# a16z/jolt

Hardware: AMD Instinct MI355X
Metric: prover trace cycles/sec (sha3-shaped synthetic trace, sumcheck + HyperKZG hot path) (higher is better)
Workload: dtype u256 (BN254 Fr / Fq, 8x u32 Montgomery limbs; integer, bit-exact)

## Files before the change

### jolt_amd/csrc/rw_matrix.hip

```cpp
#include <algorithm>
#include <vector>

#include "ctx.hpp"
#include "ints.hpp"
#include "onehot.hpp"
#include "poly_kernels.hip.h"

using namespace jolt;

int32_t jolt_internal_table_new(jolt_ctx* ctx, size_t len, jolt_table** out);
int32_t jolt_internal_bind(jolt_ctx* ctx, jolt_table* const* tables, size_t k, const Fr& r, int32_t order);
int32_t jolt_internal_eq_levels(jolt_ctx* ctx, const Fr* r, size_t n, const Fr& scale, std::vector<jolt_table*>* levels);
int32_t jolt_internal_ensure_scratch(jolt_ctx* ctx, size_t partials, size_t results);

namespace {

constexpr uint64_t kNoAccess = 0xFFFFFFFFFFFFFFFFull;

struct RwArrays {
    uint64_t* key;
    uint64_t *prev_u, *next_u;
    Fr *prev_f, *next_f;
    Fr *val, *ra;
    Fr* wa;
};

__device__ __forceinline__ uint32_t lower_bound_near(const uint64_t* __restrict__ a, uint32_t n, uint64_t x, uint32_t hint) {
    uint32_t lo, hi;
    if (a[hint] < x) {
        uint32_t prev = hint, step = 1;
        hi = n;
        for (;;) {
            const uint32_t probe = prev + step;
            if (probe >= n || probe < prev) break;
            if (a[probe] < x) { prev = probe; step <<= 1; }
            else { hi = probe; break; }
        }
        lo = prev + 1;
    } else {
        uint32_t next = hint, step = 1;
        lo = 0;
        for (;;) {
            if (next < step) break;
            const uint32_t probe = next - step;
            if (a[probe] >= x) { next = probe; step <<= 1; }
            else { lo = probe + 1; break; }
        }
        hi = next;
    }
    while (lo < hi) {
        const uint32_t mid = (lo + hi) >> 1;
        if (a[mid] < x) lo = mid + 1;
        else hi = mid;
    }
    return lo;
}

__device__ __forceinline__ Fr bind_pair(const Fr& lo, const Fr& hi, const Fr& r, int shifted) {
    return shifted ? jolt::bind_pair<true>(lo, hi, r) : jolt::bind_pair<false>(lo, hi, r);
}
__device__ __forceinline__ Fr slope_term(const Fr& val, const Fr& inc, const Fr& gamma) { return add(val, mul(gamma, add(inc, val))); }

__global__ __launch_bounds__(kBlock) void k_rw_access_flags(const uint64_t* __restrict__ addresses, uint32_t cycles, uint64_t* __restrict__ flags) {
    uint32_t j = blockIdx.x * kBlock + threadIdx.x;
    if (j < cycles) flags[j] = addresses[j] != kNoAccess ? 1ull : 0ull;
}
__global__ __launch_bounds__(kBlock) void k_rw_build(const uint64_t* __restrict__ addresses, const uint64_t* __restrict__ pre, const uint64_t* __restrict__ post,
                                                     uint32_t cycles, const uint64_t* __restrict__ pos, RwArrays o) {
    uint32_t j = blockIdx.x * kBlock + threadIdx.x;
    if (j >= cycles || addresses[j] == kNoAccess) return;
    const uint32_t p = (uint32_t)pos[j];
    o.key[p] = ((uint64_t)j << 32) | (uint32_t)addresses[j];
    o.prev_u[p] = pre[j];
    o.next_u[p] = post[j];
    st_fr(o.val + p, fr_from_u64(pre[j]));
    st_fr(o.ra + p, Fr::one());
}

struct RegCells {
    uint32_t col[3];
    uint64_t prev[3], next[3], val[3];
    uint32_t ra_kind[3];
    uint32_t wa[3];
    uint32_t len;
};
__device__ __forceinline__ RegCells reg_cells(uint32_t rs1, uint64_t rs1_val, uint32_t rs2, uint64_t rs2_val, uint32_t rd, uint64_t rd_pre, uint64_t rd_post) {
    RegCells c;
    c.len = 0;
    if (rs1 != kColdIdx) { c.col[0] = rs1; c.prev[0] = rs1_val; c.next[0] = rs1_val; c.val[0] = rs1_val; c.ra_kind[0] = 1; c.wa[0] = 0; c.len = 1; }
    if (rs2 != kColdIdx) {
        if (c.len && c.col[0] == rs2) c.ra_kind[0] = 3;
        else { const uint32_t k = c.len++; c.col[k] = rs2; c.prev[k] = rs2_val; c.next[k] = rs2_val; c.val[k] = rs2_val; c.ra_kind[k] = 2; c.wa[k] = 0; }
    }
    if (rd != kColdIdx) {
        uint32_t f = 0;
        while (f < c.len && c.col[f] != rd) ++f;
        if (f < c.len) { c.wa[f] = 1; c.next[f] = rd_post; }
        else { const uint32_t k = c.len++; c.col[k] = rd; c.prev[k] = rd_pre; c.next[k] = rd_post; c.val[k] = rd_pre; c.ra_kind[k] = 0; c.wa[k] = 1; }
    }
    return c;
}
__global__ __launch_bounds__(kBlock) void k_reg_count(const uint8_t* __restrict__ idx, uint32_t wide, uint32_t cycles, uint64_t* __restrict__ flags) {
    const uint32_t j = blockIdx.x * kBlock + threadIdx.x;
    if (j >= cycles) return;
    const uint32_t rs1 = hot_load(hot_col(idx, 0, wide), j, wide), rs2 = hot_load(hot_col(idx, cycles, wide), j, wide), rd = hot_load(hot_col(idx, 2 * (size_t)cycles, wide), j, wide);
    uint32_t count = rs1 != kColdIdx ? 1u : 0u;
    if (rs2 != kColdIdx && rs2 != rs1) count += 1;
    if (rd != kColdIdx && rd != rs1 && rd != rs2) count += 1;
    flags[j] = count;
}
__global__ __launch_bounds__(kBlock) void k_reg_build(const uint8_t* __restrict__ idx, uint32_t wide, const uint64_t* __restrict__ rs1_val, const uint64_t* __restrict__ rs2_val,
                                                      const uint64_t* __restrict__ rd_pre, const uint64_t* __restrict__ rd_post, uint32_t cycles, const uint64_t* __restrict__ pos,
                                                      Fr gamma, Fr gamma2, RwArrays o) {
    const uint32_t j = blockIdx.x * kBlock + threadIdx.x;
    if (j >= cycles) return;
    const uint32_t rs1 = hot_load(hot_col(idx, 0, wide), j, wide), rs2 = hot_load(hot_col(idx, cycles, wide), j, wide), rd = hot_load(hot_col(idx, 2 * (size_t)cycles, wide), j, wide);
    RegCells c = reg_cells(rs1, rs1_val[j], rs2, rs2_val[j], rd, rd_pre[j], rd_post[j]);
    uint32_t ord[3] = {0, 1, 2};
    for (uint32_t a = 0; a < c.len; ++a)
        for (uint32_t b = a + 1; b < c.len; ++b)
            if (c.col[ord[b]] < c.col[ord[a]]) { const uint32_t t = ord[a]; ord[a] = ord[b]; ord[b] = t; }
    const uint32_t p0 = (uint32_t)pos[j];
    for (uint32_t a = 0; a < c.len; ++a) {
        const uint32_t k = ord[a], p = p0 + a;
        o.key[p] = ((uint64_t)j << 32) | c.col[k];
        o.prev_u[p] = c.prev[k];
        o.next_u[p] = c.next[k];
        st_fr(o.val + p, fr_from_u64(c.val[k]));
        const Fr ra = c.ra_kind[k] == 0 ? Fr::zero() : (c.ra_kind[k] == 1 ? gamma : (c.ra_kind[k] == 2 ? gamma2 : add(gamma, gamma2)));
        st_fr(o.ra + p, ra);
        st_fr(o.wa + p, c.wa[k] ? Fr::one() : Fr::zero());
    }
}

constexpr int kScanItems = 4;
__global__ __launch_bounds__(kBlock) void k_scan_blocks(const uint64_t* __restrict__ in, uint32_t n, uint64_t* __restrict__ out, uint64_t* __restrict__ block_sums) {
    __shared__ uint64_t sm[kBlock];
    const uint32_t base = (blockIdx.x * kBlock + threadIdx.x) * kScanItems;
    uint64_t v[kScanItems], local = 0;
#pragma unroll
    for (int k = 0; k < kScanItems; ++k) {
        v[k] = base + k < n ? in[base + k] : 0ull;
        local += v[k];
    }
    sm[threadIdx.x] = local;
    __syncthreads();
    for (int off = 1; off < kBlock; off <<= 1) {
        uint64_t t = (int)threadIdx.x >= off ? sm[threadIdx.x - off] : 0ull;
        __syncthreads();
        sm[threadIdx.x] += t;
        __syncthreads();
    }
    uint64_t run = sm[threadIdx.x] - local;
#pragma unroll
    for (int k = 0; k < kScanItems; ++k) {
        if (base + k < n) out[base + k] = run;
        run += v[k];
    }
    if (threadIdx.x == kBlock - 1) block_sums[blockIdx.x] = sm[threadIdx.x];
}
__global__ __launch_bounds__(kBlock) void k_scan_sums(uint64_t* __restrict__ sums, uint32_t nblocks, uint64_t* __restrict__ total) {
    __shared__ uint64_t sm[kBlock];
    __shared__ uint64_t carry;
    if (threadIdx.x == 0) carry = 0;
    __syncthreads();
    for (uint32_t base = 0; base < nblocks; base += kBlock) {
        const uint32_t i = base + threadIdx.x;
        const uint64_t v = i < nblocks ? sums[i] : 0ull;
        sm[threadIdx.x] = v;
        __syncthreads();
        for (int off = 1; off < kBlock; off <<= 1) {
            uint64_t t = (int)threadIdx.x >= off ? sm[threadIdx.x - off] : 0ull;
            __syncthreads();
            sm[threadIdx.x] += t;
            __syncthreads();
        }
        if (i < nblocks) sums[i] = carry + sm[threadIdx.x] - v;
        __syncthreads();
        if (threadIdx.x == kBlock - 1) carry += sm[threadIdx.x];
        __syncthreads();
    }
    if (threadIdx.x == 0) total[0] = carry;
}
__global__ __launch_bounds__(kBlock) void k_scan_add(uint64_t* __restrict__ out, uint32_t n, const uint64_t* __restrict__ block_sums) {
    const uint32_t base = (blockIdx.x * kBlock + threadIdx.x) * kScanItems;
    const uint64_t add_ = block_sums[blockIdx.x];
#pragma unroll
    for (int k = 0; k < kScanItems; ++k)
        if (base + k < n) out[base + k] += add_;
}

__global__ __launch_bounds__(kBlock) void k_rw_cycle_match(const uint64_t* __restrict__ key, uint32_t n, uint32_t* __restrict__ sib_lb, uint32_t* __restrict__ matched,
                                                           uint64_t* __restrict__ flags) {
    uint32_t i = blockIdx.x * kBlock + threadIdx.x;
    if (i >= n) return;
    const uint64_t k = key[i], want = k ^ (1ull << 32);
    const uint32_t lb = lower_bound_near(key, n, want, i);
    const bool m = lb < n && key[lb] == want;
    const bool even = ((k >> 32) & 1) == 0;
    sib_lb[i] = lb;
    matched[i] = m ? 1u : 0u;
    flags[i] = ((even || !m) ? 1ull : 0ull) | ((even && m) ? (1ull << 32) : 0ull);
}

template <bool REG>
__global__ __launch_bounds__(kBlock) void k_rw_cycle_round(RwArrays a, uint32_t n, const uint32_t* __restrict__ sib_lb, const uint32_t* __restrict__ matched,
                                                           const Fr* __restrict__ inc, const Fr* __restrict__ e_out, const Fr* __restrict__ e_in, int in_bits, Fr gamma,
                                                           Fr* __restrict__ partials) {
    Fr acc[2] = {Fr::zero(), Fr::zero()};
    const uint32_t stride = gridDim.x * kBlock;
    for (uint32_t i = blockIdx.x * kBlock + threadIdx.x; i < n; i += stride) {
        const uint64_t k = a.key[i];
        const uint32_t row = (uint32_t)(k >> 32);
        const bool even = (row & 1) == 0, m = matched[i] != 0;
        if (!even && m) continue;
        const uint32_t pair = row >> 1;
        const Fr inc0 = ld_fr(inc + 2 * (size_t)pair), inc1 = sub(ld_fr(inc + 2 * (size_t)pair + 1), inc0);
        const Fr ra = ld_fr(a.ra + i), val = ld_fr(a.val + i);
        Fr q0, q1;
        if constexpr (REG) {
            const Fr wa = ld_fr(a.wa + i);
            if (even) {
                Fr ra_slope, wa_slope, val_slope;
                if (m) {
                    const uint32_t o = sib_lb[i];
                    ra_slope = sub(ld_fr(a.ra + o), ra);
                    wa_slope = sub(ld_fr(a.wa + o), wa);
                    val_slope = sub(ld_fr(a.val + o), val);
                } else {
                    ra_slope = neg(ra);
                    wa_slope = neg(wa);
                    val_slope = sub(fr_from_u64(a.next_u[i]), val);
                }
                q0 = add(mul(ra, val), mul(wa, add(val, inc0)));
                q1 = add(mul(ra_slope, val_slope), mul(wa_slope, add(val_slope, inc1)));
            } else {
                const Fr val_slope = sub(val, fr_from_u64(a.prev_u[i]));
                q0 = Fr::zero();
                q1 = add(mul(ra, val_slope), mul(wa, add(val_slope, inc1)));
            }
        } else if (even) {
            Fr ra_slope, val_slope;
            if (m) {
                const uint32_t o = sib_lb[i];
                ra_slope = sub(ld_fr(a.ra + o), ra);
                val_slope = sub(ld_fr(a.val + o), val);
            } else {
                ra_slope = neg(ra);
                val_slope = sub(fr_from_u64(a.next_u[i]), val);
            }
            q0 = mul(ra, slope_term(val, inc0, gamma));
            q1 = mul(ra_slope, slope_term(val_slope, inc1, gamma));
        } else {
            q0 = Fr::zero();
            q1 = mul(ra, slope_term(sub(val, fr_from_u64(a.prev_u[i])), inc1, gamma));
        }
        const Fr head = mul(ld_fr(e_out + (pair >> in_bits)), ld_fr(e_in + (pair & ((1u << in_bits) - 1))));
        acc[0] = add(acc[0], mul(head, q0));
        acc[1] = add(acc[1], mul(head, q1));
    }
    block_reduce_store<2>(acc, partials);
}

template <bool REG>
__global__ __launch_bounds__(kBlock) void k_rw_cycle_bind(RwArrays a, uint32_t n, const uint32_t* __restrict__ sib_lb, const uint32_t* __restrict__ matched,
                                                          const uint64_t* __restrict__ scan, Fr r, int shifted, RwArrays o) {
    uint32_t i = blockIdx.x * kBlock + threadIdx.x;
    if (i >= n) return;
    const uint64_t k = a.key[i];
    const uint32_t row = (uint32_t)(k >> 32), col = (uint32_t)k;
    const bool even = (row & 1) == 0, m = matched[i] != 0;
    if (!even && m) return;
    const uint64_t gkey = (uint64_t)(row & ~1u) << 32;
    const uint32_t gs = lower_bound_near(a.key, n, gkey, i), os = lower_bound_near(a.key, n, gkey | (1ull << 32), i);
    const uint64_t s_gs = gs < n ? scan[gs] : 0;
    const uint32_t out_base = (uint32_t)s_gs, m_gs = (uint32_t)(s_gs >> 32);
    const uint32_t lb = sib_lb[i];
    uint32_t pos;
    if (even) pos = out_base + (i - gs) + (lb - os) - ((uint32_t)(scan[i] >> 32) - m_gs);
    else pos = out_base + (i - os) + (lb - gs) - ((lb < n ? (uint32_t)(scan[lb] >> 32) : 0u) - m_gs);
    const Fr ra = ld_fr(a.ra + i), val = ld_fr(a.val + i);
    Fr nra, nval;
    uint64_t np, nn;
    auto lerp = [&](const Fr& lo, const Fr& hi) { return bind_pair(lo, hi, r, shifted); };
    if (even && m) {
        nra = lerp(ra, ld_fr(a.ra + lb));
        nval = lerp(val, ld_fr(a.val + lb));
        np = a.prev_u[i];
        nn = a.next_u[lb];
    } else if (even) {
        nra = lerp(ra, Fr::zero());
        nval = lerp(val, fr_from_u64(a.next_u[i]));
        np = a.prev_u[i];
        nn = a.next_u[i];
    } else {
        nra = lerp(Fr::zero(), ra);
        nval = lerp(fr_from_u64(a.prev_u[i]), val);
        np = a.prev_u[i];
        nn = a.next_u[i];
    }
    o.key[pos] = ((uint64_t)(row >> 1) << 32) | col;
    o.prev_u[pos] = np;
    o.next_u[pos] = nn;
    st_fr(o.ra + pos, nra);
    st_fr(o.val + pos, nval);
    if constexpr (REG) {
        const Fr wa = ld_fr(a.wa + i);
        st_fr(o.wa + pos, (even && m) ? lerp(wa, ld_fr(a.wa + lb)) : (even ? lerp(wa, Fr::zero()) : lerp(Fr::zero(), wa)));
    }
}

__global__ __launch_bounds__(kBlock) void k_rw_to_address_major(RwArrays a, uint32_t n) {
    uint32_t i = blockIdx.x * kBlock + threadIdx.x;
    if (i >= n) return;
    a.key[i] = (uint32_t)a.key[i];
    st_fr(a.prev_f + i, fr_from_u64(a.prev_u[i]));
    st_fr(a.next_f + i, fr_from_u64(a.next_u[i]));
}

__device__ __forceinline__ bool adr_partner(const uint64_t* __restrict__ key, uint32_t n, uint32_t i, uint32_t& other) {
    const uint64_t c = key[i];
    if ((c & 1) == 0) { other = i + 1; return i + 1 < n && key[i + 1] == c + 1; }
    other = i - 1;
    return i > 0 && key[i - 1] == c - 1;
}
__global__ __launch_bounds__(kBlock) void k_rw_address_flags(const uint64_t* __restrict__ key, uint32_t n, uint64_t* __restrict__ flags) {
    uint32_t i = blockIdx.x * kBlock + threadIdx.x;
    if (i >= n) return;
    uint32_t o;
    const bool m = adr_partner(key, n, i, o);
    flags[i] = ((key[i] & 1) == 0 || !m) ? 1ull : 0ull;
}
__global__ __launch_bounds__(kBlock) void k_rw_address_round(RwArrays a, uint32_t n, const Fr* __restrict__ val_init, const Fr* __restrict__ inc_scalar, Fr eq_eval,
                                                             Fr gamma, Fr* __restrict__ partials) {
    Fr acc[2] = {Fr::zero(), Fr::zero()};
    const Fr inc = ld_fr(inc_scalar);
    const uint32_t stride = gridDim.x * kBlock;
    for (uint32_t i = blockIdx.x * kBlock + threadIdx.x; i < n; i += stride) {
        uint32_t o;
        const bool m = adr_partner(a.key, n, i, o);
        const uint64_t c = a.key[i];
        const bool even = (c & 1) == 0;
        if (!even && m) continue;
        const Fr ra = ld_fr(a.ra + i), val = ld_fr(a.val + i);
        Fr s0, s2;
        if (even) {
            Fr ra2, val2;
            if (m) {
                const Fr ora = ld_fr(a.ra + o), oval = ld_fr(a.val + o);
                ra2 = sub(add(ora, ora), ra);
                val2 = sub(add(oval, oval), val);
            } else {
                const Fr cp = ld_fr(val_init + (c | 1));
                ra2 = neg(ra);
                val2 = sub(add(cp, cp), val);
            }
            s0 = mul(mul(eq_eval, ra), slope_term(val, inc, gamma));
            s2 = mul(mul(eq_eval, ra2), slope_term(val2, inc, gamma));
        } else {
            const Fr cp = ld_fr(val_init + (c & ~1ull));
            s0 = Fr::zero();
            s2 = mul(mul(eq_eval, add(ra, ra)), slope_term(sub(add(val, val), cp), inc, gamma));
        }
        acc[0] = add(acc[0], s0);
        acc[1] = add(acc[1], s2);
    }
    block_reduce_store<2>(acc, partials);
}
__global__ __launch_bounds__(kBlock) void k_rw_address_bind(RwArrays a, uint32_t n, const Fr* __restrict__ val_init, const uint64_t* __restrict__ scan, Fr r, int shifted,
                                                            RwArrays o) {
    uint32_t i = blockIdx.x * kBlock + threadIdx.x;
    if (i >= n) return;
    uint32_t p;
    const bool m = adr_partner(a.key, n, i, p);
    const uint64_t c = a.key[i];
    const bool even = (c & 1) == 0;
    if (!even && m) return;
    const uint32_t pos = (uint32_t)scan[i];
    auto lerp = [&](const Fr& lo, const Fr& hi) { return bind_pair(lo, hi, r, shifted); };
    const Fr ra = ld_fr(a.ra + i), val = ld_fr(a.val + i), pv = ld_fr(a.prev_f + i), nx = ld_fr(a.next_f + i);
    Fr nra, nval, npv, nnx;
    if (even && m) {
        nra = lerp(ra, ld_fr(a.ra + p));
        nval = lerp(val, ld_fr(a.val + p));
        npv = lerp(pv, ld_fr(a.prev_f + p));
        nnx = lerp(nx, ld_fr(a.next_f + p));
    } else if (even) {
        const Fr cp = ld_fr(val_init + (c | 1));
        nra = lerp(ra, Fr::zero());
        nval = lerp(val, cp);
        npv = lerp(pv, cp);
        nnx = lerp(nx, cp);
    } else {
        const Fr cp = ld_fr(val_init + (c & ~1ull));
        nra = lerp(Fr::zero(), ra);
        nval = lerp(cp, val);
        npv = lerp(cp, pv);
        nnx = lerp(cp, nx);
    }
    o.key[pos] = c >> 1;
    st_fr(o.ra + pos, nra);
    st_fr(o.val + pos, nval);
    st_fr(o.prev_f + pos, npv);
    st_fr(o.next_f + pos, nnx);
}

}

struct jolt_rw_matrix {
    jolt_ctx* ctx = nullptr;
    size_t log_t = 0, log_k = 0, round = 0;
    uint32_t n = 0, cap = 0;
    void* block = nullptr;
    RwArrays st[2];
    int cur = 0;
    uint32_t *sib_lb = nullptr, *matched = nullptr;
    uint64_t *flags = nullptr, *scan = nullptr, *block_sums = nullptr, *total = nullptr;
    uint64_t* h_total = nullptr;
    bool match_valid = false;
    bool registers = false;
    bool hold_row = false;
    std::vector<Fr> reg_ra, reg_wa, reg_val;
    Fr inc_scalar;
    jolt_table *inc = nullptr, *val_init = nullptr;
    Fr gamma;
    std::vector<Fr> w;
    Fr current_scalar;
    size_t out_len = 0, in_len = 0, e_out_bits = 0, e_in_bits = 0;
    std::vector<jolt_table*> e_out_cache, e_in_cache;
};

static int32_t rw_scan(jolt_rw_matrix* m, uint32_t n) {
    jolt_ctx* ctx = m->ctx;
    const uint32_t per = kBlock * kScanItems, nblocks = std::max<uint32_t>(1, (n + per - 1) / per);
    hipLaunchKernelGGL(k_scan_blocks, dim3(nblocks), dim3(kBlock), 0, ctx->stream, (const uint64_t*)m->flags, n, m->scan, m->block_sums);
    hipLaunchKernelGGL(k_scan_sums, dim3(1), dim3(kBlock), 0, ctx->stream, m->block_sums, nblocks, m->total);
    hipLaunchKernelGGL(k_scan_add, dim3(nblocks), dim3(kBlock), 0, ctx->stream, m->scan, n, (const uint64_t*)m->block_sums);
    JOLT_HIP_TRY(ctx, hipGetLastError());
    return JOLT_OK;
}
static int32_t rw_read_total(jolt_rw_matrix* m, uint32_t* out) {
    jolt_ctx* ctx = m->ctx;
    JOLT_HIP_TRY(ctx, hipMemcpyAsync(m->h_total, m->total, 8, hipMemcpyDeviceToHost, ctx->stream));
    JOLT_HIP_TRY(ctx, hipStreamSynchronize(ctx->stream));
    *out = (uint32_t)*m->h_total;
    return JOLT_OK;
}
static unsigned rw_grid(uint32_t n) { return std::max<unsigned>(1, (n + kBlock - 1) / kBlock); }
constexpr uint32_t kRwRoundMult = 4;

extern "C" int32_t jolt_rw_matrix_destroy(jolt_rw_matrix* m) {
    if (!m) return JOLT_OK;
    jolt_ctx* ctx = m->ctx;
    if (m->block) jolt_internal_dev_free(ctx, m->block);
    if (m->h_total) (void)hipHostFree(m->h_total);
    if (m->inc) jolt_table_free(ctx, m->inc);
    if (m->val_init) jolt_table_free(ctx, m->val_init);
    for (jolt_table* t : m->e_out_cache) jolt_table_free(ctx, t);
    for (jolt_table* t : m->e_in_cache) jolt_table_free(ctx, t);
    delete m;
    return JOLT_OK;
}

static int32_t rw_create_impl(jolt_ctx* ctx, const uint64_t* addresses, const uint64_t* pre_values, const uint64_t* post_values, bool resident, uint32_t resident_cap,
                              size_t cycles, const jolt_table* inc, const jolt_table* val_init, const jolt_fr_t* tau_low, const jolt_fr_t* gamma, jolt_rw_matrix** out) {
    if (!ctx || !addresses || !pre_values || !post_values || !inc || !val_init || !tau_low || !gamma || !out) return JOLT_ERR_INVALID_ARG;
    if (cycles < 2 || (cycles & (cycles - 1)) || cycles > ((size_t)1 << 31) || inc->len != cycles) return JOLT_ERR_SIZE_MISMATCH;
    const size_t K = val_init->len;
    if (K == 0 || (K & (K - 1)) || K > ((size_t)1 << 32)) return JOLT_ERR_SIZE_MISMATCH;
    for (size_t j = 0; j < cycles && !resident; ++j)
        if (addresses[j] != kNoAccess && addresses[j] >= K) { ctx->last_error = "RAM address outside the address space"; return JOLT_ERR_INVALID_ARG; }
    jolt_rw_matrix* m = new (std::nothrow) jolt_rw_matrix();
    if (!m) return JOLT_ERR_OOM;
    m->ctx = ctx;
    while (((size_t)1 << m->log_t) < cycles) m->log_t++;
    while (((size_t)1 << m->log_k) < K) m->log_k++;
    m->gamma = fr_from_abi(gamma);
    m->w.resize(m->log_t);
    for (size_t i = 0; i < m->log_t; ++i) m->w[i] = fr_from_abi(&tau_low[i]);
    m->current_scalar = Fr::one();
    int32_t s = fr_is_canonical(m->gamma) ? JOLT_OK : JOLT_ERR_INVALID_ARG;
    for (size_t i = 0; i < m->log_t && s == JOLT_OK; ++i) if (!fr_is_canonical(m->w[i])) s = JOLT_ERR_INVALID_ARG;
    const size_t split = m->log_t / 2, head_len = m->log_t - 1;
    m->out_len = std::min(split, head_len);
    m->in_len = head_len - m->out_len;
    m->e_out_bits = m->out_len;
    m->e_in_bits = m->in_len;
    if (s == JOLT_OK) s = jolt_internal_eq_levels(ctx, m->w.data(), m->out_len, Fr::one(), &m->e_out_cache);
    if (s == JOLT_OK) s = jolt_internal_eq_levels(ctx, m->w.data() + m->out_len, m->in_len, Fr::one(), &m->e_in_cache);
    if (s == JOLT_OK) s = jolt_table_clone(ctx, inc, &m->inc);
    if (s == JOLT_OK) s = jolt_table_clone(ctx, val_init, &m->val_init);
    const uint32_t T = (uint32_t)cycles;
    uint32_t cap = resident_cap;
    for (size_t j = 0; j < cycles && !resident; ++j) cap += addresses[j] != kNoAccess;
    m->cap = std::max<uint32_t>(cap, 1);
    const size_t scan_len = std::max<size_t>(T, m->cap);
    size_t off = 0;
    auto take = [&](size_t bytes) { size_t o = off; off += (bytes + 255) & ~(size_t)255; return o; };
    size_t o_up = take(resident ? 256 : 3 * cycles * 8);
    size_t o_st[2][8];
    for (int b = 0; b < 2; ++b) {
        o_st[b][0] = take((size_t)m->cap * 8); o_st[b][1] = take((size_t)m->cap * 8); o_st[b][2] = take((size_t)m->cap * 8);
        o_st[b][3] = take((size_t)m->cap * 32); o_st[b][4] = take((size_t)m->cap * 32); o_st[b][5] = take((size_t)m->cap * 32); o_st[b][6] = take((size_t)m->cap * 32);
        o_st[b][7] = take(256);
    }
    const size_t o_sib = take((size_t)m->cap * 4), o_match = take((size_t)m->cap * 4), o_flags = take(scan_len * 8), o_scan = take(scan_len * 8),
                 o_bs = take(((scan_len + kBlock * kScanItems - 1) / (kBlock * kScanItems) + 1) * 8), o_total = take(256);
    if (s == JOLT_OK) s = jolt_internal_dev_alloc(ctx, off, &m->block);
    if (s == JOLT_OK && hipHostMalloc((void**)&m->h_total, 64, hipHostMallocDefault) != hipSuccess) s = JOLT_ERR_HIP;
    if (s != JOLT_OK) { jolt_rw_matrix_destroy(m); return s; }
    char* base = (char*)m->block;
    for (int b = 0; b < 2; ++b) {
        m->st[b].key = (uint64_t*)(base + o_st[b][0]); m->st[b].prev_u = (uint64_t*)(base + o_st[b][1]); m->st[b].next_u = (uint64_t*)(base + o_st[b][2]);
        m->st[b].prev_f = (Fr*)(base + o_st[b][3]); m->st[b].next_f = (Fr*)(base + o_st[b][4]); m->st[b].val = (Fr*)(base + o_st[b][5]); m->st[b].ra = (Fr*)(base + o_st[b][6]);
        m->st[b].wa = (Fr*)(base + o_st[b][7]);
    }
    m->sib_lb = (uint32_t*)(base + o_sib); m->matched = (uint32_t*)(base + o_match); m->flags = (uint64_t*)(base + o_flags); m->scan = (uint64_t*)(base + o_scan);
    m->block_sums = (uint64_t*)(base + o_bs); m->total = (uint64_t*)(base + o_total);
    const uint64_t *d_addr = addresses, *d_pre = pre_values, *d_post = post_values;
    hipError_t e = hipSuccess;
    if (!resident) {
        uint64_t* up = (uint64_t*)(base + o_up);
        d_addr = up; d_pre = up + cycles; d_post = up + 2 * cycles;
        e = hipMemcpyAsync(up, addresses, cycles * 8, hipMemcpyHostToDevice, ctx->stream);
        if (e == hipSuccess) e = hipMemcpyAsync(up + cycles, pre_values, cycles * 8, hipMemcpyHostToDevice, ctx->stream);
        if (e == hipSuccess) e = hipMemcpyAsync(up + 2 * cycles, post_values, cycles * 8, hipMemcpyHostToDevice, ctx->stream);
    }
    if (e == hipSuccess) {
        hipLaunchKernelGGL(k_rw_access_flags, dim3(rw_grid(T)), dim3(kBlock), 0, ctx->stream, (const uint64_t*)d_addr, T, m->flags);
        e = hipGetLastError();
    }
    if (e == hipSuccess) s = rw_scan(m, T);
    if (e == hipSuccess && s == JOLT_OK) {
        hipLaunchKernelGGL(k_rw_build, dim3(rw_grid(T)), dim3(kBlock), 0, ctx->stream, (const uint64_t*)d_addr, (const uint64_t*)d_pre, (const uint64_t*)d_post, T,
                           (const uint64_t*)m->scan, m->st[0]);
        e = hipGetLastError();
    }
    if (e == hipSuccess && !resident) e = hipStreamSynchronize(ctx->stream);
    if (e != hipSuccess || s != JOLT_OK) {
        if (e != hipSuccess) { ctx->last_error = std::string("rw matrix: ") + hipGetErrorString(e); s = JOLT_ERR_HIP; }
        jolt_rw_matrix_destroy(m);
        return s;
    }
    m->n = cap;
    *out = m;
    return JOLT_OK;
}
extern "C" int32_t jolt_rw_matrix_create(jolt_ctx* ctx, const uint64_t* addresses, const uint64_t* pre_values, const uint64_t* post_values, size_t cycles,
                                         const jolt_table* inc, const jolt_table* val_init, const jolt_fr_t* tau_low, const jolt_fr_t* gamma, jolt_rw_matrix** out) {
    return rw_create_impl(ctx, addresses, pre_values, post_values, false, 0, cycles, inc, val_init, tau_low, gamma, out);
}
__global__ __launch_bounds__(kBlock) void k_rw_count_accesses(const uint64_t* __restrict__ addresses, uint32_t cycles, uint64_t K, uint32_t* __restrict__ counters) {
    __shared__ uint32_t s_hit[kBlock / 64], s_bad[kBlock / 64];
    uint32_t hit = 0, bad = 0;
    for (uint32_t j = blockIdx.x * kBlock + threadIdx.x; j < cycles; j += gridDim.x * kBlock) {
        const uint64_t a = addresses[j];
        hit += a != kNoAccess ? 1u : 0u;
        bad += (a != kNoAccess && a >= K) ? 1u : 0u;
    }
    for (int off = 32; off >= 1; off >>= 1) {
        hit += __shfl_xor(hit, off, 64);
        bad += __shfl_xor(bad, off, 64);
    }
    if ((threadIdx.x & 63) == 0) { s_hit[threadIdx.x >> 6] = hit; s_bad[threadIdx.x >> 6] = bad; }
    __syncthreads();
    if (threadIdx.x == 0) {
        uint32_t h = 0, b = 0;
        for (int w = 0; w < kBlock / 64; ++w) { h += s_hit[w]; b += s_bad[w]; }
        if (h) atomicAdd(&counters[0], h);
        if (b) atomicAdd(&counters[1], b);
    }
}
extern "C" int32_t jolt_rw_matrix_create_resident(jolt_ctx* ctx, const jolt_ints* addresses, const jolt_ints* pre_values, const jolt_ints* post_values,
                                                  const jolt_table* inc, const jolt_table* val_init, const jolt_fr_t* tau_low, const jolt_fr_t* gamma, jolt_rw_matrix** out) {
    if (!ctx || !addresses || !pre_values || !post_values || !val_init || !out) return JOLT_ERR_INVALID_ARG;
    if (addresses->kind != JOLT_INT_U64 || pre_values->kind != JOLT_INT_U64 || post_values->kind != JOLT_INT_U64) return JOLT_ERR_INVALID_ARG;
    const size_t cycles = addresses->count;
    if (pre_values->count != cycles || post_values->count != cycles) return JOLT_ERR_SIZE_MISMATCH;
    if (cycles < 2 || cycles > ((size_t)1 << 31)) return JOLT_ERR_SIZE_MISMATCH;
    uint32_t* d_counters = nullptr;
    JOLT_TRY(jolt_internal_dev_alloc(ctx, 256, (void**)&d_counters));
    uint32_t h_counters[2] = {0, 0};
    hipError_t e = hipMemsetAsync(d_counters, 0, 8, ctx->stream);
    if (e == hipSuccess) {
        hipLaunchKernelGGL(k_rw_count_accesses, dim3(std::min<uint32_t>(rw_grid((uint32_t)cycles), (uint32_t)ctx->num_cus * 8)), dim3(kBlock), 0, ctx->stream, (const uint64_t*)addresses->data, (uint32_t)cycles,
                           (uint64_t)val_init->len, d_counters);
        e = hipGetLastError();
    }
    if (e == hipSuccess) e = hipMemcpyAsync(h_counters, d_counters, 8, hipMemcpyDeviceToHost, ctx->stream);
    if (e == hipSuccess) e = hipStreamSynchronize(ctx->stream);
    jolt_internal_dev_free(ctx, d_counters);
    if (e != hipSuccess) { ctx->last_error = std::string("rw matrix: ") + hipGetErrorString(e); return JOLT_ERR_HIP; }
    if (h_counters[1]) { ctx->last_error = "RAM address outside the address space"; return JOLT_ERR_INVALID_ARG; }
    return rw_create_impl(ctx, (const uint64_t*)addresses->data, (const uint64_t*)pre_values->data, (const uint64_t*)post_values->data, true, h_counters[0], cycles, inc,
                          val_init, tau_low, gamma, out);
}

static int32_t rw_ingest(jolt_rw_matrix* m, const Fr& r) {
    jolt_ctx* ctx = m->ctx;
    const int shifted = fr_low_limbs_zero(r) ? 1 : 0;
    RwArrays &a = m->st[m->cur], &o = m->st[1 - m->cur];
    if (m->round < m->log_t) {
        if (m->n) {
            if (!m->match_valid) {
                hipLaunchKernelGGL(k_rw_cycle_match, dim3(rw_grid(m->n)), dim3(kBlock), 0, ctx->stream, (const uint64_t*)a.key, m->n, m->sib_lb, m->matched, m->flags);
                JOLT_HIP_TRY(ctx, hipGetLastError());
            }
            JOLT_TRY(rw_scan(m, m->n));
            if (m->registers)
                hipLaunchKernelGGL(k_rw_cycle_bind<true>, dim3(rw_grid(m->n)), dim3(kBlock), 0, ctx->stream, a, m->n, (const uint32_t*)m->sib_lb, (const uint32_t*)m->matched,
                                   (const uint64_t*)m->scan, r, shifted, o);
            else
                hipLaunchKernelGGL(k_rw_cycle_bind<false>, dim3(rw_grid(m->n)), dim3(kBlock), 0, ctx->stream, a, m->n, (const uint32_t*)m->sib_lb, (const uint32_t*)m->matched,
                                   (const uint64_t*)m->scan, r, shifted, o);
            JOLT_HIP_TRY(ctx, hipGetLastError());
            JOLT_TRY(rw_read_total(m, &m->n));
            m->cur = 1 - m->cur;
        }
        m->match_valid = false;
        JOLT_TRY(jolt_internal_bind(ctx, &m->inc, 1, r, JOLT_ORDER_LOW_TO_HIGH));
        {
            const size_t nvar = m->log_t;
            size_t current_index = nvar - m->round;
            const Fr p = m->w[current_index - 1], prod = mul(p, r);
            m->current_scalar = mul(m->current_scalar, add(add(sub(sub(Fr::one(), p), r), prod), prod));
            current_index -= 1;
            if (nvar / 2 < current_index && m->e_in_bits > 0) m->e_in_bits -= 1;
            else if (0 < current_index && m->e_out_bits > 0) m->e_out_bits -= 1;
        }
        if (m->round == m->log_t - 1 && m->hold_row) {
        } else if (m->round == m->log_t - 1 && m->registers) {
            const size_t K = (size_t)1 << m->log_k;
            m->reg_ra.assign(K, Fr::zero());
            m->reg_wa.assign(K, Fr::zero());
            m->reg_val.assign(K, Fr::zero());
            const uint32_t n = m->n;
            if (n > K) { ctx->last_error = "registers matrix: more cells than registers after the cycle rounds"; return JOLT_ERR_INVALID_ARG; }
            std::vector<uint64_t> key(n);
            std::vector<Fr> ra(n), wa(n), val(n);
            const RwArrays& c = m->st[m->cur];
            hipError_t first = hipSuccess;
            auto copy = [&](void* dst, const void* src, size_t bytes) {
                const hipError_t e = hipMemcpyAsync(dst, src, bytes, hipMemcpyDeviceToHost, ctx->stream);
                if (first == hipSuccess) first = e;
            };
            if (n) {
                copy(key.data(), c.key, (size_t)n * 8);
                copy(ra.data(), c.ra, (size_t)n * sizeof(Fr));
                copy(wa.data(), c.wa, (size_t)n * sizeof(Fr));
                copy(val.data(), c.val, (size_t)n * sizeof(Fr));
            }
            copy(&m->inc_scalar, m->inc->data(), sizeof(Fr));
            const hipError_t sync = hipStreamSynchronize(ctx->stream);
            JOLT_HIP_TRY(ctx, first);
            JOLT_HIP_TRY(ctx, sync);
            for (uint32_t i = 0; i < n; ++i) {
                const uint32_t col = (uint32_t)key[i];
                if ((key[i] >> 32) != 0 || col >= K) { ctx->last_error = "registers matrix: a cell outside the single bound row"; return JOLT_ERR_INVALID_ARG; }
                m->reg_ra[col] = ra[i]; m->reg_wa[col] = wa[i]; m->reg_val[col] = val[i];
            }
        } else if (m->round == m->log_t - 1 && m->n) {
            hipLaunchKernelGGL(k_rw_to_address_major, dim3(rw_grid(m->n)), dim3(kBlock), 0, ctx->stream, m->st[m->cur], m->n);
            JOLT_HIP_TRY(ctx, hipGetLastError());
        }
    } else if (m->registers) {
        for (std::vector<Fr>* t : {&m->reg_ra, &m->reg_wa, &m->reg_val}) {
            const size_t half = t->size() / 2;
            for (size_t y = 0; y < half; ++y) (*t)[y] = add((*t)[2 * y], mul(r, sub((*t)[2 * y + 1], (*t)[2 * y])));
            t->resize(half);
        }
    } else {
        if (m->n) {
            hipLaunchKernelGGL(k_rw_address_flags, dim3(rw_grid(m->n)), dim3(kBlock), 0, ctx->stream, (const uint64_t*)a.key, m->n, m->flags);
            JOLT_HIP_TRY(ctx, hipGetLastError());
            JOLT_TRY(rw_scan(m, m->n));
            hipLaunchKernelGGL(k_rw_address_bind, dim3(rw_grid(m->n)), dim3(kBlock), 0, ctx->stream, a, m->n, (const Fr*)m->val_init->data(), (const uint64_t*)m->scan, r,
                               shifted, o);
            JOLT_HIP_TRY(ctx, hipGetLastError());
            JOLT_TRY(rw_read_total(m, &m->n));
            m->cur = 1 - m->cur;
        }
        JOLT_TRY(jolt_internal_bind(ctx, &m->val_init, 1, r, JOLT_ORDER_LOW_TO_HIGH));
    }
    m->round += 1;
    return JOLT_OK;
}

extern "C" int32_t jolt_rw_matrix_prove_round(jolt_rw_matrix* m, const jolt_fr_t* bind, jolt_fr_t* evals_out, jolt_fr_t* aux_out) {
    if (!m || !evals_out) return JOLT_ERR_INVALID_ARG;
    jolt_ctx* ctx = m->ctx;
    if (m->registers) { ctx->last_error = "a registers handle: use jolt_registers_rw_prove_round (this entry point ignores the wa column)"; return JOLT_ERR_INVALID_ARG; }
    if (bind) {
        Fr r = fr_from_abi(bind);
        JOLT_REQUIRE(ctx, fr_is_canonical(r), "bind challenge is not a canonical Fr");
        if (m->round >= m->log_t + m->log_k) { ctx->last_error = "rw matrix already fully bound"; return JOLT_ERR_INVALID_ARG; }
        JOLT_TRY(rw_ingest(m, r));
    }
    if (m->round >= m->log_t + m->log_k) { ctx->last_error = "prove_round on a fully bound rw matrix"; return JOLT_ERR_INVALID_ARG; }
    const int grid = (int)std::max<uint32_t>(1, std::min<uint32_t>((m->n + kBlock - 1) / kBlock, (uint32_t)ctx->num_cus * kRwRoundMult));
    JOLT_TRY(jolt_internal_ensure_scratch(ctx, (size_t)grid * 2 + 8, 8));
    RwArrays& a = m->st[m->cur];
    Fr zero = Fr::zero();
    if (m->round < m->log_t) {
        if (m->n && !m->match_valid) {
            hipLaunchKernelGGL(k_rw_cycle_match, dim3(rw_grid(m->n)), dim3(kBlock), 0, ctx->stream, (const uint64_t*)a.key, m->n, m->sib_lb, m->matched, m->flags);
            JOLT_HIP_TRY(ctx, hipGetLastError());
            m->match_valid = true;
        }
        hipLaunchKernelGGL(k_rw_cycle_round<false>, dim3(grid), dim3(kBlock), 0, ctx->stream, a, m->n, (const uint32_t*)m->sib_lb, (const uint32_t*)m->matched,
                           (const Fr*)m->inc->data(), (const Fr*)m->e_out_cache[m->e_out_bits]->data(), (const Fr*)m->e_in_cache[m->e_in_bits]->data(), (int)m->e_in_bits,
                           m->gamma, ctx->d_partials);
        if (aux_out) {
            fr_to_abi(&aux_out[0], m->current_scalar);
            fr_to_abi(&aux_out[1], m->w[m->log_t - m->round - 1]);
            fr_to_abi(&aux_out[2], zero);
        }
    } else {
        hipLaunchKernelGGL(k_rw_address_round, dim3(grid), dim3(kBlock), 0, ctx->stream, a, m->n, (const Fr*)m->val_init->data(), (const Fr*)m->inc->data(),
                           m->current_scalar, m->gamma, ctx->d_partials);
        if (aux_out) for (int k = 0; k < 3; ++k) fr_to_abi(&aux_out[k], zero);
    }
    JOLT_HIP_TRY(ctx, hipGetLastError());
    hipLaunchKernelGGL(k_reduce_partials, dim3(1), dim3(kBlock), 0, ctx->stream, (const Fr*)ctx->d_partials, grid, 2, ctx->d_results);
    JOLT_HIP_TRY(ctx, hipGetLastError());
    JOLT_HIP_TRY(ctx, hipMemcpyAsync(ctx->h_results, ctx->d_results, 2 * sizeof(Fr), hipMemcpyDeviceToHost, ctx->stream));
    JOLT_HIP_TRY(ctx, hipStreamSynchronize(ctx->stream));
    std::memcpy(evals_out, ctx->h_results, 2 * sizeof(Fr));
    return JOLT_OK;
}

extern "C" int32_t jolt_rw_matrix_finish(jolt_rw_matrix* m, const jolt_fr_t* bind) {
    if (!m || !bind) return JOLT_ERR_INVALID_ARG;
    Fr r = fr_from_abi(bind);
    JOLT_REQUIRE(m->ctx, fr_is_canonical(r), "bind challenge is not a canonical Fr");
    if (m->round + 1 != m->log_t + m->log_k) { m->ctx->last_error = "finish_rounds before the last round"; return JOLT_ERR_INVALID_ARG; }
    return rw_ingest(m, r);
}

extern "C" int32_t jolt_rw_matrix_final_values(jolt_rw_matrix* m, jolt_fr_t* out) {
    if (!m || !out) return JOLT_ERR_INVALID_ARG;
    jolt_ctx* ctx = m->ctx;
    if (m->registers) { ctx->last_error = "a registers handle: use jolt_registers_rw_final_values (no val_init column here)"; return JOLT_ERR_INVALID_ARG; }
    if (m->round != m->log_t + m->log_k) return JOLT_ERR_NOT_FULLY_BOUND;
    Fr vals[3];
    if (m->n) {
        JOLT_HIP_TRY(ctx, hipMemcpyAsync(&vals[0], m->st[m->cur].ra, sizeof(Fr), hipMemcpyDeviceToHost, ctx->stream));
        JOLT_HIP_TRY(ctx, hipMemcpyAsync(&vals[1], m->st[m->cur].val, sizeof(Fr), hipMemcpyDeviceToHost, ctx->stream));
    } else {
        vals[0] = Fr::zero();
        JOLT_HIP_TRY(ctx, hipMemcpyAsync(&vals[1], m->val_init->data(), sizeof(Fr), hipMemcpyDeviceToHost, ctx->stream));
    }
    JOLT_HIP_TRY(ctx, hipMemcpyAsync(&vals[2], m->inc->data(), sizeof(Fr), hipMemcpyDeviceToHost, ctx->stream));
    JOLT_HIP_TRY(ctx, hipStreamSynchronize(ctx->stream));
    for (int k = 0; k < 3; ++k) fr_to_abi(&out[k], vals[k]);
    fr_to_abi(&out[3], m->current_scalar);
    return JOLT_OK;
}

extern "C" int32_t jolt_rw_matrix_len(const jolt_rw_matrix* m, size_t* entries) {
    if (!m || !entries) return JOLT_ERR_INVALID_ARG;
    *entries = m->n;
    return JOLT_OK;
}

extern "C" int32_t jolt_rw_matrix_hold_row(jolt_rw_matrix* m) {
    if (!m || m->round != 0) return JOLT_ERR_INVALID_ARG;
    m->hold_row = true;
    return JOLT_OK;
}
extern "C" int32_t jolt_rw_matrix_bind(jolt_rw_matrix* m, const jolt_fr_t* bind) {
    if (!m || !bind) return JOLT_ERR_INVALID_ARG;
    const Fr r = fr_from_abi(bind);
    JOLT_REQUIRE(m->ctx, fr_is_canonical(r), "bind challenge is not a canonical Fr");
    if (m->round >= m->log_t + m->log_k || (m->hold_row && m->round >= m->log_t)) { m->ctx->last_error = "rw matrix already bound"; return JOLT_ERR_INVALID_ARG; }
    return rw_ingest(m, r);
}
extern "C" int32_t jolt_rw_matrix_export_row(jolt_rw_matrix* m, size_t cap, uint64_t* cols, uint64_t* prev, uint64_t* next, jolt_fr_t* val, jolt_fr_t* ra, jolt_fr_t* wa,
                                             jolt_fr_t* inc_out, jolt_fr_t* scalar_out, size_t* n_out) {
    if (!m || !cols || !prev || !next || !val || !ra || !inc_out || !scalar_out || !n_out || (m->registers && !wa)) return JOLT_ERR_INVALID_ARG;
    jolt_ctx* ctx = m->ctx;
    if (!m->hold_row || m->round != m->log_t) { ctx->last_error = "export_row: a held matrix after its last cycle round"; return JOLT_ERR_INVALID_ARG; }
    const uint32_t n = m->n;
    *n_out = n;
    if (n > cap) return JOLT_ERR_SIZE_MISMATCH;
    const RwArrays& a = m->st[m->cur];
    std::vector<uint64_t> key(n);
    hipError_t first = hipSuccess;
    auto copy = [&](void* dst, const void* src, size_t bytes) {
        const hipError_t e = bytes ? hipMemcpyAsync(dst, src, bytes, hipMemcpyDeviceToHost, ctx->stream) : hipSuccess;
        if (first == hipSuccess) first = e;
    };
    copy(key.data(), a.key, (size_t)n * 8);
    copy(prev, a.prev_u, (size_t)n * 8);
    copy(next, a.next_u, (size_t)n * 8);
    copy(val, a.val, (size_t)n * sizeof(Fr));
    copy(ra, a.ra, (size_t)n * sizeof(Fr));
    if (m->registers) copy(wa, a.wa, (size_t)n * sizeof(Fr));
    Fr inc;
    copy(&inc, m->inc->data(), sizeof(Fr));
    const hipError_t sync = hipStreamSynchronize(ctx->stream);
    JOLT_HIP_TRY(ctx, first);
    JOLT_HIP_TRY(ctx, sync);
    for (uint32_t i = 0; i < n; ++i) {
        if (key[i] >> 32) { ctx->last_error = "export_row: a cell outside the single bound row"; return JOLT_ERR_INVALID_ARG; }
        cols[i] = (uint32_t)key[i];
    }
    fr_to_abi(inc_out, inc);
    fr_to_abi(scalar_out, m->current_scalar);
    return JOLT_OK;
}

extern "C" int32_t jolt_rw_matrix_create_merged(jolt_ctx* ctx, int32_t registers, size_t log_rows, size_t log_k, size_t n, const uint64_t* rows, const uint64_t* cols,
                                                const uint64_t* prev, const uint64_t* next, const jolt_fr_t* val, const jolt_fr_t* ra, const jolt_fr_t* wa, const jolt_fr_t* inc,
                                                const jolt_table* val_init, const jolt_fr_t* w, const jolt_fr_t* scalar, const jolt_fr_t* gamma, jolt_rw_matrix** out) {
    if (!ctx || !inc || !w || !scalar || !gamma || !out || (n && (!rows || !cols || !prev || !next || !val || !ra))) return JOLT_ERR_INVALID_ARG;
    if ((registers && n && !wa) || (!registers && !val_init)) return JOLT_ERR_INVALID_ARG;
    if (log_rows < 1 || log_rows > 16 || log_k > 32 || n >= ((size_t)1 << 31)) return JOLT_ERR_UNSUPPORTED;
    if (registers && log_k > 8) return JOLT_ERR_SIZE_MISMATCH;
    if (!registers && val_init->len != ((size_t)1 << log_k)) return JOLT_ERR_SIZE_MISMATCH;
    std::vector<uint64_t> key(n);
    for (size_t i = 0; i < n; ++i) {
        if (rows[i] >> log_rows || cols[i] >> log_k) { ctx->last_error = "merged rw matrix: a cell outside the matrix"; return JOLT_ERR_INVALID_ARG; }
        key[i] = (rows[i] << 32) | cols[i];
        if (i && key[i] <= key[i - 1]) { ctx->last_error = "merged rw matrix: cells must come in (row, column) order"; return JOLT_ERR_INVALID_ARG; }
    }
    jolt_rw_matrix* m = new (std::nothrow) jolt_rw_matrix();
    if (!m) return JOLT_ERR_OOM;
    m->ctx = ctx;
    m->registers = registers != 0;
    m->log_t = log_rows;
    m->log_k = log_k;
    m->gamma = fr_from_abi(gamma);
    m->current_scalar = fr_from_abi(scalar);
    m->w.resize(log_rows);
    for (size_t i = 0; i < log_rows; ++i) m->w[i] = fr_from_abi(&w[i]);
    int32_t s = fr_is_canonical(m->gamma) && fr_is_canonical(m->current_scalar) ? JOLT_OK : JOLT_ERR_INVALID_ARG;
    for (size_t i = 0; i < log_rows && s == JOLT_OK; ++i) if (!fr_is_canonical(m->w[i])) s = JOLT_ERR_INVALID_ARG;
    const size_t split = m->log_t / 2, head_len = m->log_t - 1;
    m->out_len = std::min(split, head_len);
    m->in_len = head_len - m->out_len;
    m->e_out_bits = m->out_len;
    m->e_in_bits = m->in_len;
    if (s == JOLT_OK) s = jolt_internal_eq_levels(ctx, m->w.data(), m->out_len, Fr::one(), &m->e_out_cache);
    if (s == JOLT_OK) s = jolt_internal_eq_levels(ctx, m->w.data() + m->out_len, m->in_len, Fr::one(), &m->e_in_cache);
    if (s == JOLT_OK) s = jolt_table_upload(ctx, inc, (size_t)1 << log_rows, &m->inc);
    if (s == JOLT_OK && !registers) s = jolt_table_clone(ctx, val_init, &m->val_init);
    m->cap = (uint32_t)std::max<size_t>(n, 1);
    const size_t scan_len = std::max<size_t>((size_t)1 << log_rows, m->cap);
    size_t off = 0;
    auto take = [&](size_t bytes) { size_t o = off; off += (bytes + 255) & ~(size_t)255; return o; };
    size_t o_st[2][8];
    for (int b = 0; b < 2; ++b) {
        o_st[b][0] = take((size_t)m->cap * 8); o_st[b][1] = take((size_t)m->cap * 8); o_st[b][2] = take((size_t)m->cap * 8);
        o_st[b][3] = take(registers ? 256 : (size_t)m->cap * 32); o_st[b][4] = take(registers ? 256 : (size_t)m->cap * 32);
        o_st[b][5] = take((size_t)m->cap * 32); o_st[b][6] = take((size_t)m->cap * 32); o_st[b][7] = take(registers ? (size_t)m->cap * 32 : 256);
    }
    const size_t o_sib = take((size_t)m->cap * 4), o_match = take((size_t)m->cap * 4), o_flags = take(scan_len * 8), o_scan = take(scan_len * 8),
                 o_bs = take(((scan_len + kBlock * kScanItems - 1) / (kBlock * kScanItems) + 1) * 8), o_total = take(256);
    if (s == JOLT_OK) s = jolt_internal_dev_alloc(ctx, off, &m->block);
    if (s == JOLT_OK && hipHostMalloc((void**)&m->h_total, 64, hipHostMallocDefault) != hipSuccess) s = JOLT_ERR_HIP;
    if (s != JOLT_OK) { jolt_rw_matrix_destroy(m); return s; }
    char* base = (char*)m->block;
    for (int b = 0; b < 2; ++b) {
        m->st[b].key = (uint64_t*)(base + o_st[b][0]); m->st[b].prev_u = (uint64_t*)(base + o_st[b][1]); m->st[b].next_u = (uint64_t*)(base + o_st[b][2]);
        m->st[b].prev_f = registers ? nullptr : (Fr*)(base + o_st[b][3]); m->st[b].next_f = registers ? nullptr : (Fr*)(base + o_st[b][4]);
        m->st[b].val = (Fr*)(base + o_st[b][5]); m->st[b].ra = (Fr*)(base + o_st[b][6]); m->st[b].wa = (Fr*)(base + o_st[b][7]);
    }
    m->sib_lb = (uint32_t*)(base + o_sib); m->matched = (uint32_t*)(base + o_match); m->flags = (uint64_t*)(base + o_flags); m->scan = (uint64_t*)(base + o_scan);
    m->block_sums = (uint64_t*)(base + o_bs); m->total = (uint64_t*)(base + o_total);
    hipError_t first = hipSuccess;
    auto up = [&](void* dst, const void* src, size_t bytes) {
        const hipError_t e = bytes ? hipMemcpyAsync(dst, src, bytes, hipMemcpyHostToDevice, ctx->stream) : hipSuccess;
        if (first == hipSuccess) first = e;
    };
    up(m->st[0].key, key.data(), n * 8);
    up(m->st[0].prev_u, prev, n * 8);
    up(m->st[0].next_u, next, n * 8);
    up(m->st[0].val, val, n * sizeof(Fr));
    up(m->st[0].ra, ra, n * sizeof(Fr));
    if (registers) up(m->st[0].wa, wa, n * sizeof(Fr));
    const hipError_t sync = hipStreamSynchronize(ctx->stream);
    if (first != hipSuccess || sync != hipSuccess) {
        ctx->last_error = std::string("merged rw matrix: ") + hipGetErrorString(first != hipSuccess ? first : sync);
        jolt_rw_matrix_destroy(m);
        return JOLT_ERR_HIP;
    }
    m->n = (uint32_t)n;
    *out = m;
    return JOLT_OK;
}

extern "C" int32_t jolt_rw_matrix_download(jolt_rw_matrix* m, uint64_t* rows, uint64_t* cols, jolt_fr_t* val, jolt_fr_t* ra, jolt_fr_t* prev, jolt_fr_t* next) {
    if (!m || !rows || !cols || !val || !ra || !prev || !next) return JOLT_ERR_INVALID_ARG;
    jolt_ctx* ctx = m->ctx;
    if (m->registers) { ctx->last_error = "a registers handle: use jolt_registers_rw_download (no prev / next field columns here)"; return JOLT_ERR_INVALID_ARG; }
    const uint32_t n = m->n;
    if (!n) return JOLT_OK;
    const RwArrays& a = m->st[m->cur];
    const bool address_major = m->round >= m->log_t;
    std::vector<uint64_t> key(n), pu(n), nu(n);
    JOLT_HIP_TRY(ctx, hipMemcpyAsync(key.data(), a.key, (size_t)n * 8, hipMemcpyDeviceToHost, ctx->stream));
    JOLT_HIP_TRY(ctx, hipMemcpyAsync(val, a.val, (size_t)n * 32, hipMemcpyDeviceToHost, ctx->stream));
    JOLT_HIP_TRY(ctx, hipMemcpyAsync(ra, a.ra, (size_t)n * 32, hipMemcpyDeviceToHost, ctx->stream));
    if (address_major) {
        JOLT_HIP_TRY(ctx, hipMemcpyAsync(prev, a.prev_f, (size_t)n * 32, hipMemcpyDeviceToHost, ctx->stream));
        JOLT_HIP_TRY(ctx, hipMemcpyAsync(next, a.next_f, (size_t)n * 32, hipMemcpyDeviceToHost, ctx->stream));
    } else {
        JOLT_HIP_TRY(ctx, hipMemcpyAsync(pu.data(), a.prev_u, (size_t)n * 8, hipMemcpyDeviceToHost, ctx->stream));
        JOLT_HIP_TRY(ctx, hipMemcpyAsync(nu.data(), a.next_u, (size_t)n * 8, hipMemcpyDeviceToHost, ctx->stream));
    }
    JOLT_HIP_TRY(ctx, hipStreamSynchronize(ctx->stream));
    for (uint32_t i = 0; i < n; ++i) {
        rows[i] = address_major ? 0 : key[i] >> 32;
        cols[i] = address_major ? key[i] : (uint32_t)key[i];
        if (!address_major) {
            Fr p = fr_from_u64(pu[i]), q = fr_from_u64(nu[i]);
            fr_to_abi(&prev[i], p);
            fr_to_abi(&next[i], q);
        }
    }
    return JOLT_OK;
}

extern "C" int32_t jolt_registers_rw_create(jolt_ctx* ctx, const jolt_onehot* regs, const jolt_ints* rs1_val, const jolt_ints* rs2_val, const jolt_ints* rd_pre,
                                            const jolt_ints* rd_post, const jolt_table* inc, const jolt_fr_t* r_cycle, const jolt_fr_t* gamma, jolt_rw_matrix** out) {
    if (!ctx || !regs || !rs1_val || !rs2_val || !rd_pre || !rd_post || !inc || !r_cycle || !gamma || !out) return JOLT_ERR_INVALID_ARG;
    if (regs->n_polys != 3) { ctx->last_error = "registers columns: a hot-index source with the three columns rs1, rs2, rd"; return JOLT_ERR_INVALID_ARG; }
    const size_t cycles = regs->cycles, K = regs->k;
    for (const jolt_ints* c : {rs1_val, rs2_val, rd_pre, rd_post}) {
        if (c->kind != JOLT_INT_U64) return JOLT_ERR_INVALID_ARG;
        if (c->count != cycles) return JOLT_ERR_SIZE_MISMATCH;
    }
    if (cycles < 2 || (cycles & (cycles - 1)) || cycles > ((size_t)1 << 30) || inc->len != cycles) return JOLT_ERR_SIZE_MISMATCH;
    if (K == 0 || (K & (K - 1)) || K > 256) return JOLT_ERR_SIZE_MISMATCH;
    jolt_rw_matrix* m = new (std::nothrow) jolt_rw_matrix();
    if (!m) return JOLT_ERR_OOM;
    m->ctx = ctx;
    m->registers = true;
    while (((size_t)1 << m->log_t) < cycles) m->log_t++;
    while (((size_t)1 << m->log_k) < K) m->log_k++;
    m->gamma = fr_from_abi(gamma);
    m->w.resize(m->log_t);
    for (size_t i = 0; i < m->log_t; ++i) m->w[i] = fr_from_abi(&r_cycle[i]);
    m->current_scalar = Fr::one();
    int32_t s = fr_is_canonical(m->gamma) ? JOLT_OK : JOLT_ERR_INVALID_ARG;
    for (size_t i = 0; i < m->log_t && s == JOLT_OK; ++i) if (!fr_is_canonical(m->w[i])) s = JOLT_ERR_INVALID_ARG;
    const size_t split = m->log_t / 2, head_len = m->log_t - 1;
    m->out_len = std::min(split, head_len);
    m->in_len = head_len - m->out_len;
    m->e_out_bits = m->out_len;
    m->e_in_bits = m->in_len;
    if (s == JOLT_OK) s = jolt_internal_eq_levels(ctx, m->w.data(), m->out_len, Fr::one(), &m->e_out_cache);
    if (s == JOLT_OK) s = jolt_internal_eq_levels(ctx, m->w.data() + m->out_len, m->in_len, Fr::one(), &m->e_in_cache);
    if (s == JOLT_OK) s = jolt_table_clone(ctx, inc, &m->inc);
    const uint32_t T = (uint32_t)cycles;
    const size_t scan_len0 = T;
    uint64_t *d_flags0 = nullptr;
    if (s == JOLT_OK) s = jolt_internal_dev_alloc(ctx, (2 * scan_len0 + ((scan_len0 + kBlock * kScanItems - 1) / (kBlock * kScanItems) + 1) + 32) * 8, (void**)&d_flags0);
    if (s == JOLT_OK && hipHostMalloc((void**)&m->h_total, 64, hipHostMallocDefault) != hipSuccess) s = JOLT_ERR_HIP;
    if (s != JOLT_OK) { if (d_flags0) jolt_internal_dev_free(ctx, d_flags0); jolt_rw_matrix_destroy(m); return s; }
    m->flags = d_flags0; m->scan = d_flags0 + scan_len0; m->block_sums = m->scan + scan_len0; m->total = m->block_sums + ((scan_len0 + kBlock * kScanItems - 1) / (kBlock * kScanItems) + 1);
    hipLaunchKernelGGL(k_reg_count, dim3(rw_grid(T)), dim3(kBlock), 0, ctx->stream, (const uint8_t*)regs->idx, regs->wide, T, m->flags);
    s = hipGetLastError() == hipSuccess ? rw_scan(m, T) : JOLT_ERR_HIP;
    uint32_t cap = 0;
    if (s == JOLT_OK) s = rw_read_total(m, &cap);
    if (s != JOLT_OK) { jolt_internal_dev_free(ctx, d_flags0); m->flags = m->scan = m->block_sums = m->total = nullptr; jolt_rw_matrix_destroy(m); return s; }
    m->cap = std::max<uint32_t>(cap, 1);
    const size_t scan_len = std::max<size_t>(T, m->cap);
    size_t off = 0;
    auto take = [&](size_t bytes) { size_t o = off; off += (bytes + 255) & ~(size_t)255; return o; };
    size_t o_st[2][6];
    for (int b = 0; b < 2; ++b) {
        o_st[b][0] = take((size_t)m->cap * 8); o_st[b][1] = take((size_t)m->cap * 8); o_st[b][2] = take((size_t)m->cap * 8);
        o_st[b][3] = take((size_t)m->cap * 32); o_st[b][4] = take((size_t)m->cap * 32); o_st[b][5] = take((size_t)m->cap * 32);
    }
    const size_t o_sib = take((size_t)m->cap * 4), o_match = take((size_t)m->cap * 4), o_flags = take(scan_len * 8), o_scan = take(scan_len * 8),
                 o_bs = take(((scan_len + kBlock * kScanItems - 1) / (kBlock * kScanItems) + 1) * 8), o_total = take(256);
    s = jolt_internal_dev_alloc(ctx, off, &m->block);
    if (s != JOLT_OK) { jolt_internal_dev_free(ctx, d_flags0); m->flags = m->scan = m->block_sums = m->total = nullptr; jolt_rw_matrix_destroy(m); return s; }
    char* base = (char*)m->block;
    for (int b = 0; b < 2; ++b) {
        m->st[b].key = (uint64_t*)(base + o_st[b][0]); m->st[b].prev_u = (uint64_t*)(base + o_st[b][1]); m->st[b].next_u = (uint64_t*)(base + o_st[b][2]);
        m->st[b].val = (Fr*)(base + o_st[b][3]); m->st[b].ra = (Fr*)(base + o_st[b][4]); m->st[b].wa = (Fr*)(base + o_st[b][5]);
        m->st[b].prev_f = nullptr; m->st[b].next_f = nullptr;
    }
    const uint64_t* pos = m->scan;
    hipLaunchKernelGGL(k_reg_build, dim3(rw_grid(T)), dim3(kBlock), 0, ctx->stream, (const uint8_t*)regs->idx, regs->wide, (const uint64_t*)rs1_val->data, (const uint64_t*)rs2_val->data,
                       (const uint64_t*)rd_pre->data, (const uint64_t*)rd_post->data, T, pos, m->gamma, mul(m->gamma, m->gamma), m->st[0]);
    hipError_t e = hipGetLastError();
    jolt_internal_dev_free(ctx, d_flags0);
    m->sib_lb = (uint32_t*)(base + o_sib); m->matched = (uint32_t*)(base + o_match); m->flags = (uint64_t*)(base + o_flags); m->scan = (uint64_t*)(base + o_scan);
    m->block_sums = (uint64_t*)(base + o_bs); m->total = (uint64_t*)(base + o_total);
    if (e != hipSuccess) { ctx->last_error = std::string("registers matrix: ") + hipGetErrorString(e); jolt_rw_matrix_destroy(m); return JOLT_ERR_HIP; }
    m->n = cap;
    *out = m;
    return JOLT_OK;
}

extern "C" int32_t jolt_registers_rw_prove_round(jolt_rw_matrix* m, const jolt_fr_t* bind, jolt_fr_t* evals_out, jolt_fr_t* aux_out) {
    if (!m || !evals_out || !m->registers) return JOLT_ERR_INVALID_ARG;
    jolt_ctx* ctx = m->ctx;
    if (bind) {
        Fr r = fr_from_abi(bind);
        JOLT_REQUIRE(ctx, fr_is_canonical(r), "bind challenge is not a canonical Fr");
        if (m->round >= m->log_t + m->log_k) { ctx->last_error = "registers matrix already fully bound"; return JOLT_ERR_INVALID_ARG; }
        JOLT_TRY(rw_ingest(m, r));
    }
    if (m->round >= m->log_t + m->log_k) { ctx->last_error = "prove_round on a fully bound registers matrix"; return JOLT_ERR_INVALID_ARG; }
    const Fr zero = Fr::zero();
    for (int k = 0; k < 4; ++k) fr_to_abi(&evals_out[k], zero);
    if (aux_out) for (int k = 0; k < 3; ++k) fr_to_abi(&aux_out[k], zero);
    if (m->round < m->log_t) {
        const int grid = (int)std::max<uint32_t>(1, std::min<uint32_t>((m->n + kBlock - 1) / kBlock, (uint32_t)ctx->num_cus * kRwRoundMult));
        JOLT_TRY(jolt_internal_ensure_scratch(ctx, (size_t)grid * 2 + 8, 8));
        RwArrays& a = m->st[m->cur];
        if (m->n && !m->match_valid) {
            hipLaunchKernelGGL(k_rw_cycle_match, dim3(rw_grid(m->n)), dim3(kBlock), 0, ctx->stream, (const uint64_t*)a.key, m->n, m->sib_lb, m->matched, m->flags);
            JOLT_HIP_TRY(ctx, hipGetLastError());
            m->match_valid = true;
        }
        hipLaunchKernelGGL(k_rw_cycle_round<true>, dim3(grid), dim3(kBlock), 0, ctx->stream, a, m->n, (const uint32_t*)m->sib_lb, (const uint32_t*)m->matched, (const Fr*)m->inc->data(),
                           (const Fr*)m->e_out_cache[m->e_out_bits]->data(), (const Fr*)m->e_in_cache[m->e_in_bits]->data(), (int)m->e_in_bits, m->gamma, ctx->d_partials);
        JOLT_HIP_TRY(ctx, hipGetLastError());
        hipLaunchKernelGGL(k_reduce_partials, dim3(1), dim3(kBlock), 0, ctx->stream, (const Fr*)ctx->d_partials, grid, 2, ctx->d_results);
        JOLT_HIP_TRY(ctx, hipGetLastError());
        JOLT_HIP_TRY(ctx, hipMemcpyAsync(ctx->h_results, ctx->d_results, 2 * sizeof(Fr), hipMemcpyDeviceToHost, ctx->stream));
        JOLT_HIP_TRY(ctx, hipStreamSynchronize(ctx->stream));
        std::memcpy(evals_out, ctx->h_results, 2 * sizeof(Fr));
        if (aux_out) {
            fr_to_abi(&aux_out[0], m->current_scalar);
            fr_to_abi(&aux_out[1], m->w[m->log_t - m->round - 1]);
        }
        return JOLT_OK;
    }
    Fr ev[4] = {zero, zero, zero, zero};
    const size_t half = m->reg_ra.size() / 2;
    for (size_t y = 0; y < half; ++y) {
        Fr ra_t = m->reg_ra[2 * y], wa_t = m->reg_wa[2 * y], val_t = m->reg_val[2 * y];
        const Fr ra_m = sub(m->reg_ra[2 * y + 1], ra_t), wa_m = sub(m->reg_wa[2 * y + 1], wa_t), val_m = sub(m->reg_val[2 * y + 1], val_t);
        for (int t = 0; t < 4; ++t) {
            ev[t] = add(ev[t], add(mul(wa_t, add(m->inc_scalar, val_t)), mul(ra_t, val_t)));
            ra_t = add(ra_t, ra_m); wa_t = add(wa_t, wa_m); val_t = add(val_t, val_m);
        }
    }
    for (int t = 0; t < 4; ++t) fr_to_abi(&evals_out[t], mul(m->current_scalar, ev[t]));
    return JOLT_OK;
}

extern "C" int32_t jolt_registers_rw_final_values(jolt_rw_matrix* m, jolt_fr_t* out) {
    if (!m || !out || !m->registers) return JOLT_ERR_INVALID_ARG;
    if (m->round != m->log_t + m->log_k) return JOLT_ERR_NOT_FULLY_BOUND;
    if (m->reg_val.size() != 1) return JOLT_ERR_NOT_FULLY_BOUND;
    fr_to_abi(&out[0], m->reg_val[0]);
    fr_to_abi(&out[1], m->reg_wa[0]);
    fr_to_abi(&out[2], m->reg_ra[0]);
    fr_to_abi(&out[3], m->inc_scalar);
    fr_to_abi(&out[4], m->current_scalar);
    return JOLT_OK;
}

extern "C" int32_t jolt_registers_rw_download(jolt_rw_matrix* m, uint64_t* rows, uint64_t* cols, jolt_fr_t* val, jolt_fr_t* ra, jolt_fr_t* wa, uint64_t* prev, uint64_t* next) {
    if (!m || !m->registers || !rows || !cols || !val || !ra || !wa || !prev || !next) return JOLT_ERR_INVALID_ARG;
    jolt_ctx* ctx = m->ctx;
    const uint32_t n = m->n;
    if (!n || m->round >= m->log_t) return JOLT_OK;
    const RwArrays& a = m->st[m->cur];
    std::vector<uint64_t> key(n);
    JOLT_HIP_TRY(ctx, hipMemcpyAsync(key.data(), a.key, (size_t)n * 8, hipMemcpyDeviceToHost, ctx->stream));
    JOLT_HIP_TRY(ctx, hipMemcpyAsync(val, a.val, (size_t)n * 32, hipMemcpyDeviceToHost, ctx->stream));
    JOLT_HIP_TRY(ctx, hipMemcpyAsync(ra, a.ra, (size_t)n * 32, hipMemcpyDeviceToHost, ctx->stream));
    JOLT_HIP_TRY(ctx, hipMemcpyAsync(wa, a.wa, (size_t)n * 32, hipMemcpyDeviceToHost, ctx->stream));
    JOLT_HIP_TRY(ctx, hipMemcpyAsync(prev, a.prev_u, (size_t)n * 8, hipMemcpyDeviceToHost, ctx->stream));
    JOLT_HIP_TRY(ctx, hipMemcpyAsync(next, a.next_u, (size_t)n * 8, hipMemcpyDeviceToHost, ctx->stream));
    JOLT_HIP_TRY(ctx, hipStreamSynchronize(ctx->stream));
    for (uint32_t i = 0; i < n; ++i) { rows[i] = key[i] >> 32; cols[i] = (uint32_t)key[i]; }
    return JOLT_OK;
}
```

Baseline: 11.65 million.

## Fuse scan into single-pass ticketed kernel and keep RW counts on device

Replaces the three-kernel prefix scan (block scan, sums scan, add) with one kernel where the last block, picked by atomic tickets, scans the block sums. Build kernels add the block offset when they read positions, so the separate add pass is gone. Element counts now live on the device (n_dev), so rounds can launch without reading the count back on the host. It also adds a run-based round kernel that accumulates cells sharing a pair before multiplying by the eq head, with LDS accumulators for the registers case. These changes target fewer launches, fewer host syncs and fewer field multiplies, but add atomic and ticket complexity and upper-bound grid sizing.

```diff
diff --git a/jolt_amd/csrc/rw_matrix.hip b/jolt_amd/csrc/rw_matrix.hip
--- a/jolt_amd/csrc/rw_matrix.hip
+++ b/jolt_amd/csrc/rw_matrix.hip
@@ -1,4 +1,5 @@
 #include <algorithm>
+#include <cstdlib>
 #include <vector>
 
 #include "ctx.hpp"
@@ -16,6 +17,8 @@
 namespace {
 
 constexpr uint64_t kNoAccess = 0xFFFFFFFFFFFFFFFFull;
+constexpr int kScanItems = 4;
+constexpr uint32_t kScanTile = kBlock * kScanItems;
 
 struct RwArrays {
     uint64_t* key;
@@ -66,10 +69,10 @@
     if (j < cycles) flags[j] = addresses[j] != kNoAccess ? 1ull : 0ull;
 }
 __global__ __launch_bounds__(kBlock) void k_rw_build(const uint64_t* __restrict__ addresses, const uint64_t* __restrict__ pre, const uint64_t* __restrict__ post,
-                                                     uint32_t cycles, const uint64_t* __restrict__ pos, RwArrays o) {
+                                                     uint32_t cycles, const uint64_t* __restrict__ pos, const uint64_t* __restrict__ pos_blocks, RwArrays o) {
     uint32_t j = blockIdx.x * kBlock + threadIdx.x;
     if (j >= cycles || addresses[j] == kNoAccess) return;
-    const uint32_t p = (uint32_t)pos[j];
+    const uint32_t p = (uint32_t)(pos[j] + pos_blocks[j / kScanTile]);
     o.key[p] = ((uint64_t)j << 32) | (uint32_t)addresses[j];
     o.prev_u[p] = pre[j];
     o.next_u[p] = post[j];
@@ -111,7 +114,7 @@
 }
 __global__ __launch_bounds__(kBlock) void k_reg_build(const uint8_t* __restrict__ idx, uint32_t wide, const uint64_t* __restrict__ rs1_val, const uint64_t* __restrict__ rs2_val,
                                                       const uint64_t* __restrict__ rd_pre, const uint64_t* __restrict__ rd_post, uint32_t cycles, const uint64_t* __restrict__ pos,
-                                                      Fr gamma, Fr gamma2, RwArrays o) {
+                                                      const uint64_t* __restrict__ pos_blocks, Fr gamma, Fr gamma2, RwArrays o) {
     const uint32_t j = blockIdx.x * kBlock + threadIdx.x;
     if (j >= cycles) return;
     const uint32_t rs1 = hot_load(hot_col(idx, 0, wide), j, wide), rs2 = hot_load(hot_col(idx, cycles, wide), j, wide), rd = hot_load(hot_col(idx, 2 * (size_t)cycles, wide), j, wide);
@@ -120,7 +123,7 @@
     for (uint32_t a = 0; a < c.len; ++a)
         for (uint32_t b = a + 1; b < c.len; ++b)
             if (c.col[ord[b]] < c.col[ord[a]]) { const uint32_t t = ord[a]; ord[a] = ord[b]; ord[b] = t; }
-    const uint32_t p0 = (uint32_t)pos[j];
+    const uint32_t p0 = (uint32_t)(pos[j] + pos_blocks[j / kScanTile]);
     for (uint32_t a = 0; a < c.len; ++a) {
         const uint32_t k = ord[a], p = p0 + a;
         o.key[p] = ((uint64_t)j << 32) | c.col[k];
@@ -133,16 +136,14 @@
     }
 }
 
-constexpr int kScanItems = 4;
-__global__ __launch_bounds__(kBlock) void k_scan_blocks(const uint64_t* __restrict__ in, uint32_t n, uint64_t* __restrict__ out, uint64_t* __restrict__ block_sums) {
-    __shared__ uint64_t sm[kBlock];
-    const uint32_t base = (blockIdx.x * kBlock + threadIdx.x) * kScanItems;
-    uint64_t v[kScanItems], local = 0;
-#pragma unroll
-    for (int k = 0; k < kScanItems; ++k) {
-        v[k] = base + k < n ? in[base + k] : 0ull;
-        local += v[k];
-    }
+__device__ __forceinline__ uint32_t rw_count(const uint32_t* __restrict__ n_dev, uint32_t bound) { return n_dev ? min(*n_dev, bound) : bound; }
+
+constexpr uint32_t kScanSubTickets = 64, kScanTicketStride = 32;
+constexpr size_t kScanTicketWords = (size_t)(kScanSubTickets + 1) * kScanTicketStride;
+__device__ __forceinline__ uint64_t scan_at(const uint64_t* __restrict__ scan, const uint64_t* __restrict__ block_sums, uint32_t i) {
+    return scan[i] + block_sums[i / kScanTile];
+}
+__device__ __forceinline__ uint64_t block_scan_inclusive(uint64_t local, uint64_t* sm) {
     sm[threadIdx.x] = local;
     __syncthreads();
     for (int off = 1; off < kBlock; off <<= 1) {
@@ -151,47 +152,70 @@
         sm[threadIdx.x] += t;
         __syncthreads();
     }
-    uint64_t run = sm[threadIdx.x] - local;
+    return sm[threadIdx.x];
+}
+__global__ __launch_bounds__(kBlock) void k_scan(const uint64_t* __restrict__ in, const uint32_t* __restrict__ n_dev, uint32_t bound, uint64_t* __restrict__ out,
+                                                 uint64_t* __restrict__ block_sums, uint32_t* __restrict__ tickets, uint64_t* __restrict__ total, uint32_t* __restrict__ n_out) {
+    __shared__ uint64_t sm[kBlock];
+    __shared__ uint32_t s_last;
+    const uint32_t n = rw_count(n_dev, bound);
+    const uint32_t base = (blockIdx.x * kBlock + threadIdx.x) * kScanItems;
+    uint64_t v[kScanItems], local = 0;
+#pragma unroll
+    for (int k = 0; k < kScanItems; ++k) {
+        v[k] = base + k < n ? in[base + k] : 0ull;
+        local += v[k];
+    }
+    const uint64_t incl = block_scan_inclusive(local, sm);
+    uint64_t run = incl - local;
 #pragma unroll
     for (int k = 0; k < kScanItems; ++k) {
         if (base + k < n) out[base + k] = run;
         run += v[k];
     }
-    if (threadIdx.x == kBlock - 1) block_sums[blockIdx.x] = sm[threadIdx.x];
-}
-__global__ __launch_bounds__(kBlock) void k_scan_sums(uint64_t* __restrict__ sums, uint32_t nblocks, uint64_t* __restrict__ total) {
-    __shared__ uint64_t sm[kBlock];
-    __shared__ uint64_t carry;
-    if (threadIdx.x == 0) carry = 0;
+    if (threadIdx.x == kBlock - 1) {
+        __hip_atomic_store(block_sums + blockIdx.x, incl, __ATOMIC_RELAXED, __HIP_MEMORY_SCOPE_AGENT);
+        wait_stores_acked();
+    }
     __syncthreads();
-    for (uint32_t base = 0; base < nblocks; base += kBlock) {
-        const uint32_t i = base + threadIdx.x;
-        const uint64_t v = i < nblocks ? sums[i] : 0ull;
-        sm[threadIdx.x] = v;
-        __syncthreads();
-        for (int off = 1; off < kBlock; off <<= 1) {
-            uint64_t t = (int)threadIdx.x >= off ? sm[threadIdx.x - off] : 0ull;
-            __syncthreads();
-            sm[threadIdx.x] += t;
-            __syncthreads();
-        }
-        if (i < nblocks) sums[i] = carry + sm[threadIdx.x] - v;
-        __syncthreads();
-        if (threadIdx.x == kBlock - 1) carry += sm[threadIdx.x];
-        __syncthreads();
-    }
-    if (threadIdx.x == 0) total[0] = carry;
-}
-__global__ __launch_bounds__(kBlock) void k_scan_add(uint64_t* __restrict__ out, uint32_t n, const uint64_t* __restrict__ block_sums) {
-    const uint32_t base = (blockIdx.x * kBlock + threadIdx.x) * kScanItems;
-    const uint64_t add_ = block_sums[blockIdx.x];
-#pragma unroll
-    for (int k = 0; k < kScanItems; ++k)
-        if (base + k < n) out[base + k] += add_;
-}
-
-__global__ __launch_bounds__(kBlock) void k_rw_cycle_match(const uint64_t* __restrict__ key, uint32_t n, uint32_t* __restrict__ sib_lb, uint32_t* __restrict__ matched,
-                                                           uint64_t* __restrict__ flags) {
+    const uint32_t nblocks = gridDim.x;
+    if (threadIdx.x == 0) {
+        uint32_t last = 0;
+        if (nblocks <= kScanSubTickets) {
+            last = atomicAdd(tickets, 1u) == nblocks - 1 ? 1u : 0u;
+        } else {
+            const uint32_t r = blockIdx.x % kScanSubTickets, in_sub = (nblocks - r + kScanSubTickets - 1) / kScanSubTickets;
+            uint32_t* sub = tickets + (size_t)(1 + r) * kScanTicketStride;
+            if (atomicAdd(sub, 1u) == in_sub - 1) {
+                st_u32_agent(sub, 0u);
+                wait_stores_acked();
+                last = atomicAdd(tickets, 1u) == kScanSubTickets - 1 ? 1u : 0u;
+            }
+        }
+        s_last = last;
+    }
+    __syncthreads();
+    if (!s_last) return;
+    const uint32_t per = (nblocks + kBlock - 1) / kBlock, lo = min(threadIdx.x * per, nblocks), hi = min(lo + per, nblocks);
+    uint64_t mine = 0;
+    for (uint32_t b = lo; b < hi; ++b) mine += __hip_atomic_load(block_sums + b, __ATOMIC_RELAXED, __HIP_MEMORY_SCOPE_AGENT);
+    __syncthreads();
+    const uint64_t upto = block_scan_inclusive(mine, sm);
+    uint64_t carry = upto - mine;
+    for (uint32_t b = lo; b < hi; ++b) {
+        const uint64_t s = __hip_atomic_load(block_sums + b, __ATOMIC_RELAXED, __HIP_MEMORY_SCOPE_AGENT);
+        block_sums[b] = carry;
+        carry += s;
+    }
+    if (threadIdx.x == kBlock - 1) {
+        if (total) total[0] = upto;
+        if (n_out) n_out[0] = (uint32_t)upto;
+    }
+    if (threadIdx.x == 0) st_u32_agent(tickets, 0u);
+}
+__global__ __launch_bounds__(kBlock) void k_rw_cycle_match(const uint64_t* __restrict__ key, const uint32_t* __restrict__ n_dev, uint32_t bound, uint32_t* __restrict__ sib_lb,
+                                                           uint32_t* __restrict__ matched, uint64_t* __restrict__ flags) {
+    const uint32_t n = rw_count(n_dev, bound);
     uint32_t i = blockIdx.x * kBlock + threadIdx.x;
     if (i >= n) return;
     const uint64_t k = key[i], want = k ^ (1ull << 32);
@@ -204,67 +228,162 @@
 }
 
 template <bool REG>
-__global__ __launch_bounds__(kBlock) void k_rw_cycle_round(RwArrays a, uint32_t n, const uint32_t* __restrict__ sib_lb, const uint32_t* __restrict__ matched,
-                                                           const Fr* __restrict__ inc, const Fr* __restrict__ e_out, const Fr* __restrict__ e_in, int in_bits, Fr gamma,
-                                                           Fr* __restrict__ partials) {
-    Fr acc[2] = {Fr::zero(), Fr::zero()};
-    const uint32_t stride = gridDim.x * kBlock;
-    for (uint32_t i = blockIdx.x * kBlock + threadIdx.x; i < n; i += stride) {
-        const uint64_t k = a.key[i];
-        const uint32_t row = (uint32_t)(k >> 32);
-        const bool even = (row & 1) == 0, m = matched[i] != 0;
-        if (!even && m) continue;
-        const uint32_t pair = row >> 1;
-        const Fr inc0 = ld_fr(inc + 2 * (size_t)pair), inc1 = sub(ld_fr(inc + 2 * (size_t)pair + 1), inc0);
-        const Fr ra = ld_fr(a.ra + i), val = ld_fr(a.val + i);
-        Fr q0, q1;
-        if constexpr (REG) {
-            const Fr wa = ld_fr(a.wa + i);
-            if (even) {
-                Fr ra_slope, wa_slope, val_slope;
-                if (m) {
-                    const uint32_t o = sib_lb[i];
-                    ra_slope = sub(ld_fr(a.ra + o), ra);
-                    wa_slope = sub(ld_fr(a.wa + o), wa);
-                    val_slope = sub(ld_fr(a.val + o), val);
-                } else {
-                    ra_slope = neg(ra);
-                    wa_slope = neg(wa);
-                    val_slope = sub(fr_from_u64(a.next_u[i]), val);
-                }
-                q0 = add(mul(ra, val), mul(wa, add(val, inc0)));
-                q1 = add(mul(ra_slope, val_slope), mul(wa_slope, add(val_slope, inc1)));
-            } else {
-                const Fr val_slope = sub(val, fr_from_u64(a.prev_u[i]));
-                q0 = Fr::zero();
-                q1 = add(mul(ra, val_slope), mul(wa, add(val_slope, inc1)));
-            }
-        } else if (even) {
-            Fr ra_slope, val_slope;
+__device__ __forceinline__ void rw_cell_evals(const RwArrays& a, uint32_t i, bool even, bool m, const uint32_t* __restrict__ sib_lb, const Fr& inc0, const Fr& inc1,
+                                              const Fr& gamma, Fr& q0, Fr& q1) {
+    const Fr ra = ld_fr(a.ra + i), val = ld_fr(a.val + i);
+    if constexpr (REG) {
+        const Fr wa = ld_fr(a.wa + i);
+        if (even) {
+            Fr ra_slope, wa_slope, val_slope;
             if (m) {
                 const uint32_t o = sib_lb[i];
                 ra_slope = sub(ld_fr(a.ra + o), ra);
+                wa_slope = sub(ld_fr(a.wa + o), wa);
                 val_slope = sub(ld_fr(a.val + o), val);
             } else {
                 ra_slope = neg(ra);
+                wa_slope = neg(wa);
                 val_slope = sub(fr_from_u64(a.next_u[i]), val);
             }
-            q0 = mul(ra, slope_term(val, inc0, gamma));
-            q1 = mul(ra_slope, slope_term(val_slope, inc1, gamma));
+            q0 = add(mul(ra, val), mul(wa, add(val, inc0)));
+            q1 = add(mul(ra_slope, val_slope), mul(wa_slope, add(val_slope, inc1)));
         } else {
+            const Fr val_slope = sub(val, fr_from_u64(a.prev_u[i]));
             q0 = Fr::zero();
-            q1 = mul(ra, slope_term(sub(val, fr_from_u64(a.prev_u[i])), inc1, gamma));
-        }
-        const Fr head = mul(ld_fr(e_out + (pair >> in_bits)), ld_fr(e_in + (pair & ((1u << in_bits) - 1))));
-        acc[0] = add(acc[0], mul(head, q0));
-        acc[1] = add(acc[1], mul(head, q1));
+            q1 = add(mul(ra, val_slope), mul(wa, add(val_slope, inc1)));
+        }
+    } else if (even) {
+        Fr ra_slope, val_slope;
+        if (m) {
+            const uint32_t o = sib_lb[i];
+            ra_slope = sub(ld_fr(a.ra + o), ra);
+            val_slope = sub(ld_fr(a.val + o), val);
+        } else {
+            ra_slope = neg(ra);
+            val_slope = sub(fr_from_u64(a.next_u[i]), val);
+        }
+        q0 = mul(ra, slope_term(val, inc0, gamma));
+        q1 = mul(ra_slope, slope_term(val_slope, inc1, gamma));
+    } else {
+        q0 = Fr::zero();
+        q1 = mul(ra, slope_term(sub(val, fr_from_u64(a.prev_u[i])), inc1, gamma));
+    }
+}
+constexpr uint32_t kRwRun = 4;
+template <bool REG, bool BY_RUNS>
+__global__ __launch_bounds__(kBlock) void k_rw_cycle_round(RwArrays a, const uint32_t* __restrict__ n_dev, uint32_t bound, const uint32_t* __restrict__ sib_lb,
+                                                           const uint32_t* __restrict__ matched, const Fr* __restrict__ inc, const Fr* __restrict__ e_out,
+                                                           const Fr* __restrict__ e_in, int in_bits, Fr gamma, Fr* __restrict__ partials) {
+    const uint32_t n = rw_count(n_dev, bound);
+    Fr acc[2] = {Fr::zero(), Fr::zero()};
+    constexpr bool ACC_LDS = BY_RUNS && REG;
+    __shared__ uint32_t s_acc[ACC_LDS ? 2 : 1][ACC_LDS ? 8 : 1][ACC_LDS ? kBlock : 1];
+    if constexpr (ACC_LDS) {
+        for (int t = 0; t < 2; ++t)
+#pragma unroll
+            for (int k = 0; k < 8; ++k) s_acc[t][k][threadIdx.x] = 0u;
+    }
+    if constexpr (BY_RUNS) {
+        constexpr uint32_t kNoPair = 0xFFFFFFFFu;
+        const uint32_t tiles = (n + kBlock * kRwRun - 1) / (kBlock * kRwRun);
+        for (uint32_t tile = blockIdx.x; tile < tiles; tile += gridDim.x) {
+            const uint32_t base = (tile * kBlock + threadIdx.x) * kRwRun;
+            uint32_t cur = kNoPair;
+            Fr s0, s1;
+            auto flush = [&]() {
+                const Fr head = mul(ld_fr(e_out + (cur >> in_bits)), ld_fr(e_in + (cur & ((1u << in_bits) - 1))));
+                if constexpr (ACC_LDS) {
+                    for (int t = 0; t < 2; ++t) {
+                        Fr v;
+#pragma unroll
+                        for (int k = 0; k < 8; ++k) v.l[k] = s_acc[t][k][threadIdx.x];
+                        v = add(v, mul(head, t ? s1 : s0));
+#pragma unroll
+                        for (int k = 0; k < 8; ++k) s_acc[t][k][threadIdx.x] = v.l[k];
+                    }
+                } else {
+                    acc[0] = add(acc[0], mul(head, s0));
+                    acc[1] = add(acc[1], mul(head, s1));
+                }
+            };
+#pragma unroll 1
+            for (uint32_t c = 0; c < kRwRun; ++c) {
+                const uint32_t i = base + c;
+                if (i >= n) break;
+                const uint32_t row = (uint32_t)(a.key[i] >> 32);
+                const bool even = (row & 1) == 0, m = matched[i] != 0;
+                if (!even && m) continue;
+                const uint32_t pair = row >> 1;
+                if (pair != cur) {
+                    if (cur != kNoPair) flush();
+                    cur = pair;
+                    s0 = Fr::zero();
+                    s1 = Fr::zero();
+                }
+                const Fr inc0 = ld_fr(inc + 2 * (size_t)pair), inc1 = sub(ld_fr(inc + 2 * (size_t)pair + 1), inc0);
+                Fr q0, q1;
+                rw_cell_evals<REG>(a, i, even, m, sib_lb, inc0, inc1, gamma, q0, q1);
+                s0 = add(s0, q0);
+                s1 = add(s1, q1);
+            }
+            if (cur != kNoPair) flush();
+        }
+    } else {
+        const uint32_t stride = gridDim.x * kBlock;
+        for (uint32_t i = blockIdx.x * kBlock + threadIdx.x; i < n; i += stride) {
+            const uint32_t row = (uint32_t)(a.key[i] >> 32);
+            const bool even = (row & 1) == 0, m = matched[i] != 0;
+            if (!even && m) continue;
+            const uint32_t pair = row >> 1;
+            const Fr inc0 = ld_fr(inc + 2 * (size_t)pair), inc1 = sub(ld_fr(inc + 2 * (size_t)pair + 1), inc0);
+            Fr q0, q1;
+            rw_cell_evals<REG>(a, i, even, m, sib_lb, inc0, inc1, gamma, q0, q1);
+            const Fr head = mul(ld_fr(e_out + (pair >> in_bits)), ld_fr(e_in + (pair & ((1u << in_bits) - 1))));
+            acc[0] = add(acc[0], mul(head, q0));
+            acc[1] = add(acc[1], mul(head, q1));
+        }
+    }
+    if constexpr (ACC_LDS) {
+        for (int t = 0; t < 2; ++t)
+#pragma unroll
+            for (int k = 0; k < 8; ++k) acc[t].l[k] = s_acc[t][k][threadIdx.x];
     }
     block_reduce_store<2>(acc, partials);
 }
+__global__ __launch_bounds__(kBlock) void k_rw_reduce(const Fr* __restrict__ partials, int nblocks, const uint32_t* __restrict__ n_dev, Fr* __restrict__ out) {
+    __shared__ Fr sm[kBlock / 64];
+    const int lane = threadIdx.x & 63, wave = threadIdx.x >> 6;
+    for (int t = 0; t < 2; ++t) {
+        Fr s = Fr::zero();
+        for (int b = threadIdx.x; b < nblocks; b += kBlock) s = add(s, ld_fr(partials + (size_t)b * 2 + t));
+#pragma unroll
+        for (int off = 32; off >= 1; off >>= 1) {
+            Fr o;
+#pragma unroll
+            for (int k = 0; k < 8; ++k) o.l[k] = __shfl_xor(s.l[k], off, 64);
+            s = add(s, o);
+        }
+        if (lane == 0) sm[wave] = s;
+        __syncthreads();
+        if (threadIdx.x == 0) {
+            Fr r = sm[0];
+            for (int w = 1; w < kBlock / 64; ++w) r = add(r, sm[w]);
+            st_fr(out + t, r);
+        }
+        __syncthreads();
+    }
+    if (threadIdx.x == 0) {
+        Fr c = Fr::zero();
+        c.l[0] = *n_dev;
+        st_fr(out + 2, c);
+    }
+}
 
 template <bool REG>
-__global__ __launch_bounds__(kBlock) void k_rw_cycle_bind(RwArrays a, uint32_t n, const uint32_t* __restrict__ sib_lb, const uint32_t* __restrict__ matched,
-                                                          const uint64_t* __restrict__ scan, Fr r, int shifted, RwArrays o) {
+__global__ __launch_bounds__(kBlock) void k_rw_cycle_bind(RwArrays a, const uint32_t* __restrict__ n_dev, uint32_t bound, const uint32_t* __restrict__ sib_lb,
+                                                          const uint32_t* __restrict__ matched, const uint64_t* __restrict__ scan, const uint64_t* __restrict__ block_sums, Fr r,
+                                                          int shifted, RwArrays o) {
+    const uint32_t n = rw_count(n_dev, bound);
     uint32_t i = blockIdx.x * kBlock + threadIdx.x;
     if (i >= n) return;
     const uint64_t k = a.key[i];
@@ -273,12 +392,12 @@
     if (!even && m) return;
     const uint64_t gkey = (uint64_t)(row & ~1u) << 32;
     const uint32_t gs = lower_bound_near(a.key, n, gkey, i), os = lower_bound_near(a.key, n, gkey | (1ull << 32), i);
-    const uint64_t s_gs = gs < n ? scan[gs] : 0;
+    const uint64_t s_gs = gs < n ? scan_at(scan, block_sums, gs) : 0;
     const uint32_t out_base = (uint32_t)s_gs, m_gs = (uint32_t)(s_gs >> 32);
     const uint32_t lb = sib_lb[i];
     uint32_t pos;
-    if (even) pos = out_base + (i - gs) + (lb - os) - ((uint32_t)(scan[i] >> 32) - m_gs);
-    else pos = out_base + (i - os) + (lb - gs) - ((lb < n ? (uint32_t)(scan[lb] >> 32) : 0u) - m_gs);
+    if (even) pos = out_base + (i - gs) + (lb - os) - ((uint32_t)(scan_at(scan, block_sums, i) >> 32) - m_gs);
+    else pos = out_base + (i - os) + (lb - gs) - ((lb < n ? (uint32_t)(scan_at(scan, block_sums, lb) >> 32) : 0u) - m_gs);
     const Fr ra = ld_fr(a.ra + i), val = ld_fr(a.val + i);
     Fr nra, nval;
     uint64_t np, nn;
@@ -310,7 +429,8 @@
     }
 }
 
-__global__ __launch_bounds__(kBlock) void k_rw_to_address_major(RwArrays a, uint32_t n) {
+__global__ __launch_bounds__(kBlock) void k_rw_to_address_major(RwArrays a, const uint32_t* __restrict__ n_dev, uint32_t bound) {
+    const uint32_t n = rw_count(n_dev, bound);
     uint32_t i = blockIdx.x * kBlock + threadIdx.x;
     if (i >= n) return;
     a.key[i] = (uint32_t)a.key[i];
@@ -324,15 +444,17 @@
     other = i - 1;
     return i > 0 && key[i - 1] == c - 1;
 }
-__global__ __launch_bounds__(kBlock) void k_rw_address_flags(const uint64_t* __restrict__ key, uint32_t n, uint64_t* __restrict__ flags) {
+__global__ __launch_bounds__(kBlock) void k_rw_address_flags(const uint64_t* __restrict__ key, const uint32_t* __restrict__ n_dev, uint32_t bound, uint64_t* __restrict__ flags) {
+    const uint32_t n = rw_count(n_dev, bound);
     uint32_t i = blockIdx.x * kBlock + threadIdx.x;
     if (i >= n) return;
     uint32_t o;
     const bool m = adr_partner(key, n, i, o);
     flags[i] = ((key[i] & 1) == 0 || !m) ? 1ull : 0ull;
 }
-__global__ __launch_bounds__(kBlock) void k_rw_address_round(RwArrays a, uint32_t n, const Fr* __restrict__ val_init, const Fr* __restrict__ inc_scalar, Fr eq_eval,
-                                                             Fr gamma, Fr* __restrict__ partials) {
+__global__ __launch_bounds__(kBlock) void k_rw_address_round(RwArrays a, const uint32_t* __restrict__ n_dev, uint32_t bound, const Fr* __restrict__ val_init,
+                                                             const Fr* __restrict__ inc_scalar, Fr eq_eval, Fr gamma, Fr* __restrict__ partials) {
+    const uint32_t n = rw_count(n_dev, bound);
     Fr acc[2] = {Fr::zero(), Fr::zero()};
     const Fr inc = ld_fr(inc_scalar);
     const uint32_t stride = gridDim.x * kBlock;
@@ -367,8 +489,9 @@
     }
     block_reduce_store<2>(acc, partials);
 }
-__global__ __launch_bounds__(kBlock) void k_rw_address_bind(RwArrays a, uint32_t n, const Fr* __restrict__ val_init, const uint64_t* __restrict__ scan, Fr r, int shifted,
-                                                            RwArrays o) {
+__global__ __launch_bounds__(kBlock) void k_rw_address_bind(RwArrays a, const uint32_t* __restrict__ n_dev, uint32_t bound, const Fr* __restrict__ val_init,
+                                                            const uint64_t* __restrict__ scan, const uint64_t* __restrict__ block_sums, Fr r, int shifted, RwArrays o) {
+    const uint32_t n = rw_count(n_dev, bound);
     uint32_t i = blockIdx.x * kBlock + threadIdx.x;
     if (i >= n) return;
     uint32_t p;
@@ -376,7 +499,7 @@
     const uint64_t c = a.key[i];
     const bool even = (c & 1) == 0;
     if (!even && m) return;
-    const uint32_t pos = (uint32_t)scan[i];
+    const uint32_t pos = (uint32_t)scan_at(scan, block_sums, i);
     auto lerp = [&](const Fr& lo, const Fr& hi) { return bind_pair(lo, hi, r, shifted); };
     const Fr ra = ld_fr(a.ra + i), val = ld_fr(a.val + i), pv = ld_fr(a.prev_f + i), nx = ld_fr(a.next_f + i);
     Fr nra, nval, npv, nnx;
@@ -411,11 +534,14 @@
     jolt_ctx* ctx = nullptr;
     size_t log_t = 0, log_k = 0, round = 0;
     uint32_t n = 0, cap = 0;
+    bool n_exact = true;
+    uint32_t run_cells = 0;
     void* block = nullptr;
     RwArrays st[2];
     int cur = 0;
     uint32_t *sib_lb = nullptr, *matched = nullptr;
     uint64_t *flags = nullptr, *scan = nullptr, *block_sums = nullptr, *total = nullptr;
+    uint32_t *ncount = nullptr, *tickets = nullptr;
     uint64_t* h_total = nullptr;
     bool match_valid = false;
     bool registers = false;
@@ -430,12 +556,17 @@
     std::vector<jolt_table*> e_out_cache, e_in_cache;
 };
 
-static int32_t rw_scan(jolt_rw_matrix* m, uint32_t n) {
+constexpr size_t kRwTotalBytes = 256 + kScanTicketWords * 4;
+static hipError_t rw_total_area(jolt_rw_matrix* m, uint64_t* area) {
+    m->total = area;
+    m->ncount = (uint32_t*)area + 16;
+    m->tickets = (uint32_t*)area + 64;
+    return hipMemsetAsync(area, 0, kRwTotalBytes, m->ctx->stream);
+}
+static int32_t rw_scan(jolt_rw_matrix* m, const uint32_t* n_dev, uint32_t bound, uint32_t* n_out) {
     jolt_ctx* ctx = m->ctx;
-    const uint32_t per = kBlock * kScanItems, nblocks = std::max<uint32_t>(1, (n + per - 1) / per);
-    hipLaunchKernelGGL(k_scan_blocks, dim3(nblocks), dim3(kBlock), 0, ctx->stream, (const uint64_t*)m->flags, n, m->scan, m->block_sums);
-    hipLaunchKernelGGL(k_scan_sums, dim3(1), dim3(kBlock), 0, ctx->stream, m->block_sums, nblocks, m->total);
-    hipLaunchKernelGGL(k_scan_add, dim3(nblocks), dim3(kBlock), 0, ctx->stream, m->scan, n, (const uint64_t*)m->block_sums);
+    const uint32_t nblocks = std::max<uint32_t>(1, (bound + kScanTile - 1) / kScanTile);
+    hipLaunchKernelGGL(k_scan, dim3(nblocks), dim3(kBlock), 0, ctx->stream, (const uint64_t*)m->flags, n_dev, bound, m->scan, m->block_sums, m->tickets, m->total, n_out);
     JOLT_HIP_TRY(ctx, hipGetLastError());
     return JOLT_OK;
 }
@@ -446,8 +577,36 @@
     *out = (uint32_t)*m->h_total;
     return JOLT_OK;
 }
+static int32_t rw_exact_count(jolt_rw_matrix* m) {
+    if (m->n_exact) return JOLT_OK;
+    jolt_ctx* ctx = m->ctx;
+    JOLT_HIP_TRY(ctx, hipMemcpyAsync(m->h_total, m->ncount + m->cur, 4, hipMemcpyDeviceToHost, ctx->stream));
+    JOLT_HIP_TRY(ctx, hipStreamSynchronize(ctx->stream));
+    m->n = *(const uint32_t*)m->h_total;
+    m->n_exact = true;
+    return JOLT_OK;
+}
 static unsigned rw_grid(uint32_t n) { return std::max<unsigned>(1, (n + kBlock - 1) / kBlock); }
 constexpr uint32_t kRwRoundMult = 4;
+static uint32_t rw_run_cells(const jolt_ctx* ctx) {
+    if (const char* e = std::getenv("JOLT_RW_RUN_CELLS")) { if (std::atoll(e) > 0) return (uint32_t)std::min<long long>(std::atoll(e), 0xFFFFFFFFll); }
+    return (uint32_t)ctx->num_cus * kBlock * kRwRun;
+}
+static int rw_round_grid(const jolt_ctx* ctx, uint32_t n, bool by_runs) {
+    const uint32_t per = by_runs ? kBlock * kRwRun : kBlock;
+    return (int)std::max<uint32_t>(1, std::min<uint32_t>((n + per - 1) / per, (uint32_t)ctx->num_cus * kRwRoundMult));
+}
+static int32_t rw_round_sums(jolt_rw_matrix* m, int grid, jolt_fr_t* evals_out) {
+    jolt_ctx* ctx = m->ctx;
+    hipLaunchKernelGGL(k_rw_reduce, dim3(1), dim3(kBlock), 0, ctx->stream, (const Fr*)ctx->d_partials, grid, (const uint32_t*)(m->ncount + m->cur), ctx->d_results);
+    JOLT_HIP_TRY(ctx, hipGetLastError());
+    JOLT_HIP_TRY(ctx, hipMemcpyAsync(ctx->h_results, ctx->d_results, 3 * sizeof(Fr), hipMemcpyDeviceToHost, ctx->stream));
+    JOLT_HIP_TRY(ctx, hipStreamSynchronize(ctx->stream));
+    std::memcpy(evals_out, ctx->h_results, 2 * sizeof(Fr));
+    m->n = ctx->h_results[2].l[0];
+    m->n_exact = true;
+    return JOLT_OK;
+}
 
 extern "C" int32_t jolt_rw_matrix_destroy(jolt_rw_matrix* m) {
     if (!m) return JOLT_OK;
@@ -473,6 +632,7 @@
     jolt_rw_matrix* m = new (std::nothrow) jolt_rw_matrix();
     if (!m) return JOLT_ERR_OOM;
     m->ctx = ctx;
+    m->run_cells = rw_run_cells(ctx);
     while (((size_t)1 << m->log_t) < cycles) m->log_t++;
     while (((size_t)1 << m->log_k) < K) m->log_k++;
     m->gamma = fr_from_abi(gamma);
@@ -505,7 +665,7 @@
         o_st[b][7] = take(256);
     }
     const size_t o_sib = take((size_t)m->cap * 4), o_match = take((size_t)m->cap * 4), o_flags = take(scan_len * 8), o_scan = take(scan_len * 8),
-                 o_bs = take(((scan_len + kBlock * kScanItems - 1) / (kBlock * kScanItems) + 1) * 8), o_total = take(256);
+                 o_bs = take(((scan_len + kScanTile - 1) / kScanTile + 1) * 8), o_total = take(kRwTotalBytes);
     if (s == JOLT_OK) s = jolt_internal_dev_alloc(ctx, off, &m->block);
     if (s == JOLT_OK && hipHostMalloc((void**)&m->h_total, 64, hipHostMallocDefault) != hipSuccess) s = JOLT_ERR_HIP;
     if (s != JOLT_OK) { jolt_rw_matrix_destroy(m); return s; }
@@ -516,10 +676,10 @@
         m->st[b].wa = (Fr*)(base + o_st[b][7]);
     }
     m->sib_lb = (uint32_t*)(base + o_sib); m->matched = (uint32_t*)(base + o_match); m->flags = (uint64_t*)(base + o_flags); m->scan = (uint64_t*)(base + o_scan);
-    m->block_sums = (uint64_t*)(base + o_bs); m->total = (uint64_t*)(base + o_total);
+    m->block_sums = (uint64_t*)(base + o_bs);
     const uint64_t *d_addr = addresses, *d_pre = pre_values, *d_post = post_values;
-    hipError_t e = hipSuccess;
-    if (!resident) {
+    hipError_t e = rw_total_area(m, (uint64_t*)(base + o_total));
+    if (e == hipSuccess && !resident) {
         uint64_t* up = (uint64_t*)(base + o_up);
         d_addr = up; d_pre = up + cycles; d_post = up + 2 * cycles;
         e = hipMemcpyAsync(up, addresses, cycles * 8, hipMemcpyHostToDevice, ctx->stream);
@@ -530,10 +690,10 @@
         hipLaunchKernelGGL(k_rw_access_flags, dim3(rw_grid(T)), dim3(kBlock), 0, ctx->stream, (const uint64_t*)d_addr, T, m->flags);
         e = hipGetLastError();
     }
-    if (e == hipSuccess) s = rw_scan(m, T);
+    if (e == hipSuccess) s = rw_scan(m, nullptr, T, m->ncount);
     if (e == hipSuccess && s == JOLT_OK) {
         hipLaunchKernelGGL(k_rw_build, dim3(rw_grid(T)), dim3(kBlock), 0, ctx->stream, (const uint64_t*)d_addr, (const uint64_t*)d_pre, (const uint64_t*)d_post, T,
-                           (const uint64_t*)m->scan, m->st[0]);
+                           (const uint64_t*)m->scan, (const uint64_t*)m->block_sums, m->st[0]);
         e = hipGetLastError();
     }
     if (e == hipSuccess && !resident) e = hipStreamSynchronize(ctx->stream);
@@ -600,21 +760,22 @@
     jolt_ctx* ctx = m->ctx;
     const int shifted = fr_low_limbs_zero(r) ? 1 : 0;
     RwArrays &a = m->st[m->cur], &o = m->st[1 - m->cur];
+    const uint32_t* n_dev = m->ncount + m->cur;
     if (m->round < m->log_t) {
         if (m->n) {
             if (!m->match_valid) {
-                hipLaunchKernelGGL(k_rw_cycle_match, dim3(rw_grid(m->n)), dim3(kBlock), 0, ctx->stream, (const uint64_t*)a.key, m->n, m->sib_lb, m->matched, m->flags);
+                hipLaunchKernelGGL(k_rw_cycle_match, dim3(rw_grid(m->n)), dim3(kBlock), 0, ctx->stream, (const uint64_t*)a.key, n_dev, m->n, m->sib_lb, m->matched, m->flags);
                 JOLT_HIP_TRY(ctx, hipGetLastError());
             }
-            JOLT_TRY(rw_scan(m, m->n));
+            JOLT_TRY(rw_scan(m, n_dev, m->n, m->ncount + (1 - m->cur)));
             if (m->registers)
-                hipLaunchKernelGGL(k_rw_cycle_bind<true>, dim3(rw_grid(m->n)), dim3(kBlock), 0, ctx->stream, a, m->n, (const uint32_t*)m->sib_lb, (const uint32_t*)m->matched,
-                                   (const uint64_t*)m->scan, r, shifted, o);
+                hipLaunchKernelGGL(k_rw_cycle_bind<true>, dim3(rw_grid(m->n)), dim3(kBlock), 0, ctx->stream, a, n_dev, m->n, (const uint32_t*)m->sib_lb, (const uint32_t*)m->matched,
+                                   (const uint64_t*)m->scan, (const uint64_t*)m->block_sums, r, shifted, o);
             else
-                hipLaunchKernelGGL(k_rw_cycle_bind<false>, dim3(rw_grid(m->n)), dim3(kBlock), 0, ctx->stream, a, m->n, (const uint32_t*)m->sib_lb, (const uint32_t*)m->matched,
-                                   (const uint64_t*)m->scan, r, shifted, o);
+                hipLaunchKernelGGL(k_rw_cycle_bind<false>, dim3(rw_grid(m->n)), dim3(kBlock), 0, ctx->stream, a, n_dev, m->n, (const uint32_t*)m->sib_lb, (const uint32_t*)m->matched,
+                                   (const uint64_t*)m->scan, (const uint64_t*)m->block_sums, r, shifted, o);
             JOLT_HIP_TRY(ctx, hipGetLastError());
-            JOLT_TRY(rw_read_total(m, &m->n));
+            m->n_exact = false;
             m->cur = 1 - m->cur;
         }
         m->match_valid = false;
@@ -634,6 +795,7 @@
             m->reg_ra.assign(K, Fr::zero());
             m->reg_wa.assign(K, Fr::zero());
             m->reg_val.assign(K, Fr::zero());
+            JOLT_TRY(rw_exact_count(m));
             const uint32_t n = m->n;
             if (n > K) { ctx->last_error = "registers matrix: more cells than registers after the cycle rounds"; return JOLT_ERR_INVALID_ARG; }
             std::vector<uint64_t> key(n);
@@ -660,7 +822,7 @@
                 m->reg_ra[col] = ra[i]; m->reg_wa[col] = wa[i]; m->reg_val[col] = val[i];
             }
         } else if (m->round == m->log_t - 1 && m->n) {
-            hipLaunchKernelGGL(k_rw_to_address_major, dim3(rw_grid(m->n)), dim3(kBlock), 0, ctx->stream, m->st[m->cur], m->n);
+            hipLaunchKernelGGL(k_rw_to_address_major, dim3(rw_grid(m->n)), dim3(kBlock), 0, ctx->stream, m->st[m->cur], (const uint32_t*)(m->ncount + m->cur), m->n);
             JOLT_HIP_TRY(ctx, hipGetLastError());
         }
     } else if (m->registers) {
@@ -671,13 +833,13 @@
         }
     } else {
         if (m->n) {
-            hipLaunchKernelGGL(k_rw_address_flags, dim3(rw_grid(m->n)), dim3(kBlock), 0, ctx->stream, (const uint64_t*)a.key, m->n, m->flags);
+            hipLaunchKernelGGL(k_rw_address_flags, dim3(rw_grid(m->n)), dim3(kBlock), 0, ctx->stream, (const uint64_t*)a.key, n_dev, m->n, m->flags);
             JOLT_HIP_TRY(ctx, hipGetLastError());
-            JOLT_TRY(rw_scan(m, m->n));
-            hipLaunchKernelGGL(k_rw_address_bind, dim3(rw_grid(m->n)), dim3(kBlock), 0, ctx->stream, a, m->n, (const Fr*)m->val_init->data(), (const uint64_t*)m->scan, r,
-                               shifted, o);
+            JOLT_TRY(rw_scan(m, n_dev, m->n, m->ncount + (1 - m->cur)));
+            hipLaunchKernelGGL(k_rw_address_bind, dim3(rw_grid(m->n)), dim3(kBlock), 0, ctx->stream, a, n_dev, m->n, (const Fr*)m->val_init->data(), (const uint64_t*)m->scan,
+                               (const uint64_t*)m->block_sums, r, shifted, o);
             JOLT_HIP_TRY(ctx, hipGetLastError());
-            JOLT_TRY(rw_read_total(m, &m->n));
+            m->n_exact = false;
             m->cur = 1 - m->cur;
         }
         JOLT_TRY(jolt_internal_bind(ctx, &m->val_init, 1, r, JOLT_ORDER_LOW_TO_HIGH));
@@ -697,17 +859,21 @@
         JOLT_TRY(rw_ingest(m, r));
     }
     if (m->round >= m->log_t + m->log_k) { ctx->last_error = "prove_round on a fully bound rw matrix"; return JOLT_ERR_INVALID_ARG; }
-    const int grid = (int)std::max<uint32_t>(1, std::min<uint32_t>((m->n + kBlock - 1) / kBlock, (uint32_t)ctx->num_cus * kRwRoundMult));
+    const bool cycle = m->round < m->log_t;
+    const bool by_runs = cycle && m->n >= m->run_cells;
+    const int grid = rw_round_grid(ctx, m->n, by_runs);
     JOLT_TRY(jolt_internal_ensure_scratch(ctx, (size_t)grid * 2 + 8, 8));
     RwArrays& a = m->st[m->cur];
+    const uint32_t* n_dev = m->ncount + m->cur;
     Fr zero = Fr::zero();
-    if (m->round < m->log_t) {
+    if (cycle) {
         if (m->n && !m->match_valid) {
-            hipLaunchKernelGGL(k_rw_cycle_match, dim3(rw_grid(m->n)), dim3(kBlock), 0, ctx->stream, (const uint64_t*)a.key, m->n, m->sib_lb, m->matched, m->flags);
+            hipLaunchKernelGGL(k_rw_cycle_match, dim3(rw_grid(m->n)), dim3(kBlock), 0, ctx->stream, (const uint64_t*)a.key, n_dev, m->n, m->sib_lb, m->matched, m->flags);
             JOLT_HIP_TRY(ctx, hipGetLastError());
             m->match_valid = true;
         }
-        hipLaunchKernelGGL(k_rw_cycle_round<false>, dim3(grid), dim3(kBlock), 0, ctx->stream, a, m->n, (const uint32_t*)m->sib_lb, (const uint32_t*)m->matched,
+        auto* round = by_runs ? k_rw_cycle_round<false, true> : k_rw_cycle_round<false, false>;
+        hipLaunchKernelGGL(round, dim3(grid), dim3(kBlock), 0, ctx->stream, a, n_dev, m->n, (const uint32_t*)m->sib_lb, (const uint32_t*)m->matched,
                            (const Fr*)m->inc->data(), (const Fr*)m->e_out_cache[m->e_out_bits]->data(), (const Fr*)m->e_in_cache[m->e_in_bits]->data(), (int)m->e_in_bits,
                            m->gamma, ctx->d_partials);
         if (aux_out) {
@@ -716,17 +882,12 @@
             fr_to_abi(&aux_out[2], zero);
         }
     } else {
-        hipLaunchKernelGGL(k_rw_address_round, dim3(grid), dim3(kBlock), 0, ctx->stream, a, m->n, (const Fr*)m->val_init->data(), (const Fr*)m->inc->data(),
+        hipLaunchKernelGGL(k_rw_address_round, dim3(grid), dim3(kBlock), 0, ctx->stream, a, n_dev, m->n, (const Fr*)m->val_init->data(), (const Fr*)m->inc->data(),
                            m->current_scalar, m->gamma, ctx->d_partials);
         if (aux_out) for (int k = 0; k < 3; ++k) fr_to_abi(&aux_out[k], zero);
     }
     JOLT_HIP_TRY(ctx, hipGetLastError());
-    hipLaunchKernelGGL(k_reduce_partials, dim3(1), dim3(kBlock), 0, ctx->stream, (const Fr*)ctx->d_partials, grid, 2, ctx->d_results);
-    JOLT_HIP_TRY(ctx, hipGetLastError());
-    JOLT_HIP_TRY(ctx, hipMemcpyAsync(ctx->h_results, ctx->d_results, 2 * sizeof(Fr), hipMemcpyDeviceToHost, ctx->stream));
-    JOLT_HIP_TRY(ctx, hipStreamSynchronize(ctx->stream));
-    std::memcpy(evals_out, ctx->h_results, 2 * sizeof(Fr));
-    return JOLT_OK;
+    return rw_round_sums(m, grid, evals_out);
 }
 
 extern "C" int32_t jolt_rw_matrix_finish(jolt_rw_matrix* m, const jolt_fr_t* bind) {
@@ -759,6 +920,7 @@
 
 extern "C" int32_t jolt_rw_matrix_len(const jolt_rw_matrix* m, size_t* entries) {
     if (!m || !entries) return JOLT_ERR_INVALID_ARG;
+    JOLT_TRY(rw_exact_count(const_cast<jolt_rw_matrix*>(m)));
     *entries = m->n;
     return JOLT_OK;
 }
@@ -780,6 +942,7 @@
     if (!m || !cols || !prev || !next || !val || !ra || !inc_out || !scalar_out || !n_out || (m->registers && !wa)) return JOLT_ERR_INVALID_ARG;
     jolt_ctx* ctx = m->ctx;
     if (!m->hold_row || m->round != m->log_t) { ctx->last_error = "export_row: a held matrix after its last cycle round"; return JOLT_ERR_INVALID_ARG; }
+    JOLT_TRY(rw_exact_count(m));
     const uint32_t n = m->n;
     *n_out = n;
     if (n > cap) return JOLT_ERR_SIZE_MISMATCH;
@@ -827,6 +990,7 @@
     jolt_rw_matrix* m = new (std::nothrow) jolt_rw_matrix();
     if (!m) return JOLT_ERR_OOM;
     m->ctx = ctx;
+    m->run_cells = rw_run_cells(ctx);
     m->registers = registers != 0;
     m->log_t = log_rows;
     m->log_k = log_k;
@@ -856,7 +1020,7 @@
         o_st[b][5] = take((size_t)m->cap * 32); o_st[b][6] = take((size_t)m->cap * 32); o_st[b][7] = take(registers ? (size_t)m->cap * 32 : 256);
     }
     const size_t o_sib = take((size_t)m->cap * 4), o_match = take((size_t)m->cap * 4), o_flags = take(scan_len * 8), o_scan = take(scan_len * 8),
-                 o_bs = take(((scan_len + kBlock * kScanItems - 1) / (kBlock * kScanItems) + 1) * 8), o_total = take(256);
+                 o_bs = take(((scan_len + kScanTile - 1) / kScanTile + 1) * 8), o_total = take(kRwTotalBytes);
     if (s == JOLT_OK) s = jolt_internal_dev_alloc(ctx, off, &m->block);
     if (s == JOLT_OK && hipHostMalloc((void**)&m->h_total, 64, hipHostMallocDefault) != hipSuccess) s = JOLT_ERR_HIP;
     if (s != JOLT_OK) { jolt_rw_matrix_destroy(m); return s; }
@@ -867,8 +1031,9 @@
         m->st[b].val = (Fr*)(base + o_st[b][5]); m->st[b].ra = (Fr*)(base + o_st[b][6]); m->st[b].wa = (Fr*)(base + o_st[b][7]);
     }
     m->sib_lb = (uint32_t*)(base + o_sib); m->matched = (uint32_t*)(base + o_match); m->flags = (uint64_t*)(base + o_flags); m->scan = (uint64_t*)(base + o_scan);
-    m->block_sums = (uint64_t*)(base + o_bs); m->total = (uint64_t*)(base + o_total);
-    hipError_t first = hipSuccess;
+    m->block_sums = (uint64_t*)(base + o_bs);
+    hipError_t first = rw_total_area(m, (uint64_t*)(base + o_total));
+    if (first == hipSuccess) first = hipMemsetD32Async((hipDeviceptr_t)m->ncount, (int)(uint32_t)n, 1, ctx->stream);
     auto up = [&](void* dst, const void* src, size_t bytes) {
         const hipError_t e = bytes ? hipMemcpyAsync(dst, src, bytes, hipMemcpyHostToDevice, ctx->stream) : hipSuccess;
         if (first == hipSuccess) first = e;
@@ -894,6 +1059,7 @@
     if (!m || !rows || !cols || !val || !ra || !prev || !next) return JOLT_ERR_INVALID_ARG;
     jolt_ctx* ctx = m->ctx;
     if (m->registers) { ctx->last_error = "a registers handle: use jolt_registers_rw_download (no prev / next field columns here)"; return JOLT_ERR_INVALID_ARG; }
+    JOLT_TRY(rw_exact_count(m));
     const uint32_t n = m->n;
     if (!n) return JOLT_OK;
     const RwArrays& a = m->st[m->cur];
@@ -936,6 +1102,7 @@
     jolt_rw_matrix* m = new (std::nothrow) jolt_rw_matrix();
     if (!m) return JOLT_ERR_OOM;
     m->ctx = ctx;
+    m->run_cells = rw_run_cells(ctx);
     m->registers = true;
     while (((size_t)1 << m->log_t) < cycles) m->log_t++;
     while (((size_t)1 << m->log_k) < K) m->log_k++;
@@ -956,15 +1123,19 @@
     const uint32_t T = (uint32_t)cycles;
     const size_t scan_len0 = T;
     uint64_t *d_flags0 = nullptr;
-    if (s == JOLT_OK) s = jolt_internal_dev_alloc(ctx, (2 * scan_len0 + ((scan_len0 + kBlock * kScanItems - 1) / (kBlock * kScanItems) + 1) + 32) * 8, (void**)&d_flags0);
+    if (s == JOLT_OK) s = jolt_internal_dev_alloc(ctx, (2 * scan_len0 + ((scan_len0 + kScanTile - 1) / kScanTile + 1)) * 8 + kRwTotalBytes, (void**)&d_flags0);
     if (s == JOLT_OK && hipHostMalloc((void**)&m->h_total, 64, hipHostMallocDefault) != hipSuccess) s = JOLT_ERR_HIP;
     if (s != JOLT_OK) { if (d_flags0) jolt_internal_dev_free(ctx, d_flags0); jolt_rw_matrix_destroy(m); return s; }
-    m->flags = d_flags0; m->scan = d_flags0 + scan_len0; m->block_sums = m->scan + scan_len0; m->total = m->block_sums + ((scan_len0 + kBlock * kScanItems - 1) / (kBlock * kScanItems) + 1);
-    hipLaunchKernelGGL(k_reg_count, dim3(rw_grid(T)), dim3(kBlock), 0, ctx->stream, (const uint8_t*)regs->idx, regs->wide, T, m->flags);
-    s = hipGetLastError() == hipSuccess ? rw_scan(m, T) : JOLT_ERR_HIP;
+    m->flags = d_flags0; m->scan = d_flags0 + scan_len0; m->block_sums = m->scan + scan_len0;
+    if (rw_total_area(m, m->block_sums + ((scan_len0 + kScanTile - 1) / kScanTile + 1)) != hipSuccess) s = JOLT_ERR_HIP;
+    if (s == JOLT_OK) {
+        hipLaunchKernelGGL(k_reg_count, dim3(rw_grid(T)), dim3(kBlock), 0, ctx->stream, (const uint8_t*)regs->idx, regs->wide, T, m->flags);
+        s = hipGetLastError() == hipSuccess ? rw_scan(m, nullptr, T, nullptr) : JOLT_ERR_HIP;
+    }
     uint32_t cap = 0;
     if (s == JOLT_OK) s = rw_read_total(m, &cap);
-    if (s != JOLT_OK) { jolt_internal_dev_free(ctx, d_flags0); m->flags = m->scan = m->block_sums = m->total = nullptr; jolt_rw_matrix_destroy(m); return s; }
+    auto forget_scratch = [&]() { m->flags = m->scan = m->block_sums = m->total = nullptr; m->ncount = m->tickets = nullptr; };
+    if (s != JOLT_OK) { jolt_internal_dev_free(ctx, d_flags0); forget_scratch(); jolt_rw_matrix_destroy(m); return s; }
     m->cap = std::max<uint32_t>(cap, 1);
     const size_t scan_len = std::max<size_t>(T, m->cap);
     size_t off = 0;
@@ -975,22 +1146,24 @@
         o_st[b][3] = take((size_t)m->cap * 32); o_st[b][4] = take((size_t)m->cap * 32); o_st[b][5] = take((size_t)m->cap * 32);
     }
     const size_t o_sib = take((size_t)m->cap * 4), o_match = take((size_t)m->cap * 4), o_flags = take(scan_len * 8), o_scan = take(scan_len * 8),
-                 o_bs = take(((scan_len + kBlock * kScanItems - 1) / (kBlock * kScanItems) + 1) * 8), o_total = take(256);
+                 o_bs = take(((scan_len + kScanTile - 1) / kScanTile + 1) * 8), o_total = take(kRwTotalBytes);
     s = jolt_internal_dev_alloc(ctx, off, &m->block);
-    if (s != JOLT_OK) { jolt_internal_dev_free(ctx, d_flags0); m->flags = m->scan = m->block_sums = m->total = nullptr; jolt_rw_matrix_destroy(m); return s; }
+    if (s != JOLT_OK) { jolt_internal_dev_free(ctx, d_flags0); forget_scratch(); jolt_rw_matrix_destroy(m); return s; }
     char* base = (char*)m->block;
     for (int b = 0; b < 2; ++b) {
         m->st[b].key = (uint64_t*)(base + o_st[b][0]); m->st[b].prev_u = (uint64_t*)(base + o_st[b][1]); m->st[b].next_u = (uint64_t*)(base + o_st[b][2]);
         m->st[b].val = (Fr*)(base + o_st[b][3]); m->st[b].ra = (Fr*)(base + o_st[b][4]); m->st[b].wa = (Fr*)(base + o_st[b][5]);
         m->st[b].prev_f = nullptr; m->st[b].next_f = nullptr;
     }
-    const uint64_t* pos = m->scan;
+    const uint64_t *pos = m->scan, *pos_blocks = m->block_sums;
     hipLaunchKernelGGL(k_reg_build, dim3(rw_grid(T)), dim3(kBlock), 0, ctx->stream, (const uint8_t*)regs->idx, regs->wide, (const uint64_t*)rs1_val->data, (const uint64_t*)rs2_val->data,
-                       (const uint64_t*)rd_pre->data, (const uint64_t*)rd_post->data, T, pos, m->gamma, mul(m->gamma, m->gamma), m->st[0]);
+                       (const uint64_t*)rd_pre->data, (const uint64_t*)rd_post->data, T, pos, pos_blocks, m->gamma, mul(m->gamma, m->gamma), m->st[0]);
     hipError_t e = hipGetLastError();
     jolt_internal_dev_free(ctx, d_flags0);
     m->sib_lb = (uint32_t*)(base + o_sib); m->matched = (uint32_t*)(base + o_match); m->flags = (uint64_t*)(base + o_flags); m->scan = (uint64_t*)(base + o_scan);
-    m->block_sums = (uint64_t*)(base + o_bs); m->total = (uint64_t*)(base + o_total);
+    m->block_sums = (uint64_t*)(base + o_bs);
+    if (e == hipSuccess) e = rw_total_area(m, (uint64_t*)(base + o_total));
+    if (e == hipSuccess) e = hipMemsetD32Async((hipDeviceptr_t)m->ncount, (int)cap, 1, ctx->stream);
     if (e != hipSuccess) { ctx->last_error = std::string("registers matrix: ") + hipGetErrorString(e); jolt_rw_matrix_destroy(m); return JOLT_ERR_HIP; }
     m->n = cap;
     *out = m;
@@ -1011,22 +1184,22 @@
     for (int k = 0; k < 4; ++k) fr_to_abi(&evals_out[k], zero);
     if (aux_out) for (int k = 0; k < 3; ++k) fr_to_abi(&aux_out[k], zero);
     if (m->round < m->log_t) {
-        const int grid = (int)std::max<uint32_t>(1, std::min<uint32_t>((m->n + kBlock - 1) / kBlock, (uint32_t)ctx->num_cus * kRwRoundMult));
+        const bool by_runs = m->n >= m->run_cells;
+        const int grid = rw_round_grid(ctx, m->n, by_runs);
         JOLT_TRY(jolt_internal_ensure_scratch(ctx, (size_t)grid * 2 + 8, 8));
         RwArrays& a = m->st[m->cur];
+        const uint32_t* n_dev = m->ncount + m->cur;
         if (m->n && !m->match_valid) {
-            hipLaunchKernelGGL(k_rw_cycle_match, dim3(rw_grid(m->n)), dim3(kBlock), 0, ctx->stream, (const uint64_t*)a.key, m->n, m->sib_lb, m->matched, m->flags);
+            hipLaunchKernelGGL(k_rw_cycle_match, dim3(rw_grid(m->n)), dim3(kBlock), 0, ctx->stream, (const uint64_t*)a.key, n_dev, m->n, m->sib_lb, m->matched, m->flags);
             JOLT_HIP_TRY(ctx, hipGetLastError());
             m->match_valid = true;
         }
-        hipLaunchKernelGGL(k_rw_cycle_round<true>, dim3(grid), dim3(kBlock), 0, ctx->stream, a, m->n, (const uint32_t*)m->sib_lb, (const uint32_t*)m->matched, (const Fr*)m->inc->data(),
-                           (const Fr*)m->e_out_cache[m->e_out_bits]->data(), (const Fr*)m->e_in_cache[m->e_in_bits]->data(), (int)m->e_in_bits, m->gamma, ctx->d_partials);
+        auto* round = by_runs ? k_rw_cycle_round<true, true> : k_rw_cycle_round<true, false>;
+        hipLaunchKernelGGL(round, dim3(grid), dim3(kBlock), 0, ctx->stream, a, n_dev, m->n, (const uint32_t*)m->sib_lb, (const uint32_t*)m->matched,
+                           (const Fr*)m->inc->data(), (const Fr*)m->e_out_cache[m->e_out_bits]->data(), (const Fr*)m->e_in_cache[m->e_in_bits]->data(), (int)m->e_in_bits, m->gamma,
+                           ctx->d_partials);
         JOLT_HIP_TRY(ctx, hipGetLastError());
-        hipLaunchKernelGGL(k_reduce_partials, dim3(1), dim3(kBlock), 0, ctx->stream, (const Fr*)ctx->d_partials, grid, 2, ctx->d_results);
-        JOLT_HIP_TRY(ctx, hipGetLastError());
-        JOLT_HIP_TRY(ctx, hipMemcpyAsync(ctx->h_results, ctx->d_results, 2 * sizeof(Fr), hipMemcpyDeviceToHost, ctx->stream));
-        JOLT_HIP_TRY(ctx, hipStreamSynchronize(ctx->stream));
-        std::memcpy(evals_out, ctx->h_results, 2 * sizeof(Fr));
+        JOLT_TRY(rw_round_sums(m, grid, evals_out));
         if (aux_out) {
             fr_to_abi(&aux_out[0], m->current_scalar);
             fr_to_abi(&aux_out[1], m->w[m->log_t - m->round - 1]);
@@ -1062,8 +1235,10 @@
 extern "C" int32_t jolt_registers_rw_download(jolt_rw_matrix* m, uint64_t* rows, uint64_t* cols, jolt_fr_t* val, jolt_fr_t* ra, jolt_fr_t* wa, uint64_t* prev, uint64_t* next) {
     if (!m || !m->registers || !rows || !cols || !val || !ra || !wa || !prev || !next) return JOLT_ERR_INVALID_ARG;
     jolt_ctx* ctx = m->ctx;
+    if (m->round >= m->log_t) return JOLT_OK;
+    JOLT_TRY(rw_exact_count(m));
     const uint32_t n = m->n;
-    if (!n || m->round >= m->log_t) return JOLT_OK;
+    if (!n) return JOLT_OK;
     const RwArrays& a = m->st[m->cur];
     std::vector<uint64_t> key(n);
     JOLT_HIP_TRY(ctx, hipMemcpyAsync(key.data(), a.key, (size_t)n * 8, hipMemcpyDeviceToHost, ctx->stream));
```

After: 11.70 million (median of 3 runs). Within noise of the previous version (+0.4%).
